# Tencent/PocketFlow

Hardware: AMD Instinct MI355X
Metric: images/sec ResNet-50 INT8 quant-aware fine-tune (whole job; per GPU = value / n_gpus) (higher is better)
Workload: dtype bf16

## Files before the change

### include/pocketflow_hip.h

```cpp
#ifndef POCKETFLOW_HIP_H_
#define POCKETFLOW_HIP_H_

#include <stdint.h>

#ifdef __cplusplus
extern "C" {
#endif

enum { PF_F32 = 0, PF_BF16 = 1 };
enum { PF_ACT_NONE = 0, PF_ACT_RELU = 1, PF_ACT_RELU6 = 2 };
enum { PF_BUCKET_TENSOR = 0, PF_BUCKET_CHANNEL = 1, PF_BUCKET_SPLIT = 2 };

typedef struct PfSeg {
  int64_t offset;
  int64_t len;
  int32_t RS;
  int32_t layout;
  int32_t I, O;
  int32_t mode;
  int32_t bits;
  int32_t bucket_size;
  int32_t n_bucket;
  int64_t slot_offset;
  int64_t cb_offset;
} PfSeg;

typedef struct PfBlock { int32_t seg; int32_t chunk; int32_t row0; int32_t nrows; } PfBlock;

#define PF_CHUNK 4096

const char* pf_error_string(int err);
int pf_version(void);
int pf_tuning_reload(void);

int pf_minmax_slots_init(uint32_t* slots, int64_t n_pairs, void* stream);
int pf_minmax_tensor(const void* x, int64_t n, int dtype, int act, uint32_t* slot, void* stream);
int pf_minmax_decode(const uint32_t* slots, int64_t n_pairs, float* alpha_beta, void* stream);

int pf_uq_apply(const void* x, void* y, int64_t n, int in_dtype, int out_dtype, int act,
                const uint32_t* slot, int bits, void* stream);
int pf_act_grad(const void* g, const void* u, void* dx, int64_t n, int dtype, int act,
                void* stream);

int pf_seg_minmax(const float* w_flat, const PfSeg* segs, const PfBlock* blocks, int n_blocks,
                  uint32_t* slots, void* stream);
int pf_seg_uq_apply(const float* w_flat, void* qw_flat, int out_dtype, const PfSeg* segs,
                    const PfBlock* blocks, int n_blocks, const uint32_t* slots, void* stream);

int pf_seg_nuq_apply(const float* w_flat, void* qw_flat, int out_dtype, uint8_t* idx_flat,
                     const float* codebooks, const PfSeg* segs, const PfBlock* blocks,
                     int n_blocks, const uint32_t* slots, void* stream);
int pf_seg_nuq_codebook_grad(const void* g_flat, int g_dtype, const uint8_t* idx_flat,
                             float* dcodebooks, int64_t* acc_ws, int64_t n_codebook, const PfSeg* segs,
                             const PfBlock* blocks, int n_blocks, const uint32_t* slots, void* stream);
int pf_seg_normalize(const float* w_flat, float* xn_out, const PfSeg* segs, int seg_index,
                     const uint32_t* slots, void* stream);

int pf_ws_bkup_merge_abs(const float* var, float* bkup, const float* mask, float* abs_out,
                         int64_t n, void* stream);
int pf_kth_largest_nonneg(const float* a, int64_t n, int64_t k_desc_index, float* out,
                          uint32_t* workspace, void* stream);
int pf_ws_mask_apply(float* var, const float* bkup, float* mask, const float* thr, int64_t n,
                     void* stream);
int pf_count_nonzero(const float* x, int64_t n, unsigned long long* out, void* stream);

int pf_cp_build_mask(float* mask, const uint8_t* keep_in, const uint8_t* keep_out, int O, int RS,
                     int I, void* stream);
int pf_cp_mask_grad(float* g, const uint8_t* keep_in, const uint8_t* keep_out, int O, int RS,
                    int I, void* stream);

int pf_adam_flat(float* p, const void* g, int g_dtype, float* m, float* v, const float* mask,
                 int64_t n, int64_t n_decay, float wd, float g_scale, float lr, float beta1,
                 float beta2, float eps, float beta1_power, float beta2_power, void* stream);
int pf_momentum_flat(float* p, const void* g, int g_dtype, float* acc, const float* mask,
                     int64_t n, int64_t n_decay, float wd, float g_scale, float lr, float momentum,
                     void* stream);
int pf_adam_flat_dev(float* p, const void* g, int g_dtype, float* m, float* v, const float* mask,
                     int64_t n, int64_t n_decay, float wd, float g_scale, const float* hp, float beta1,
                     float beta2, float eps, void* stream);
int pf_momentum_flat_dev(float* p, const void* g, int g_dtype, float* acc, const float* mask,
                         int64_t n, int64_t n_decay, float wd, float g_scale, const float* hp,
                         float momentum, void* stream);
int pf_set_floats(float* dst, float a, float b, float c, float d, void* stream);

int pf_ce_distill_fwd_bwd(const void* z_s, int zs_dtype, const float* labels, const void* z_t,
                          int zt_dtype, int B, int C, float tempr, float loss_w, float* losses,
                          void* dz_s, int dz_dtype, float* row_ws, void* stream);

int pf_ce_distill_head(const void* z_s, int zs_dtype, const float* labels, const void* z_t,
                       int zt_dtype, int B, int C, float tempr, float loss_w, float* losses ,
                       void* dz_hard, void* dz_soft, int dz_dtype, float* row_ws, void* stream);
int pf_ce_combine(const void* dz_hard, const void* dz_soft, const float* g0, const float* g1, void* dz,
                  int dtype, int64_t n, void* stream);

int pf_bn_stats(const void* x, int dtype, int64_t rows, int C, float* partial ,
                int n_blocks, void* stream);
int pf_bn_finalize(const float* partial, int n_blocks, int64_t rows, int C, const void* x_row0,
                   int dtype, const float* gamma, const float* beta, float* moving_mean,
                   float* moving_var, float momentum, float eps, int training ,
                   int act, float* scale_shift , float* mean_invstd ,
                   uint32_t* slot , void* stream);
int pf_bn_act_quant_apply(const void* x, void* q, int dtype, int64_t rows, int C,
                          const float* scale_shift, int act, const uint32_t* slot, int bits,
                          int quantize, void* stream);
int pf_bn_act_quant_pool(const void* x, void* pooled, int dtype, int64_t rows, int C,
                         const float* scale_shift, int act, const uint32_t* slot, int bits,
                         int quantize, int HW, void* stream);
int pf_bn_bwd_stats_pooled(const void* g, const void* x, int dtype, int64_t rows, int C, int HW,
                           const float* scale_shift, const float* mean_invstd, int act,
                           float* partial , int n_blocks, void* stream);
int pf_bn_bwd_apply_pooled(const void* g, const void* x, void* dx, int dtype, int64_t rows, int C, int HW,
                           const float* scale_shift, const float* mean_invstd,
                           const float* dgamma, const float* dbeta, int act, void* stream);
int pf_bn_bwd_stats(const void* dq, const void* x, int dtype, int64_t rows, int C,
                    const float* scale_shift, const float* mean_invstd, int act,
                    float* partial , int n_blocks, void* stream);
int pf_bn_bwd_finalize(const float* partial, int n_blocks, int C, float* dgamma, float* dbeta,
                       void* stream);
int pf_bn_bwd_apply(const void* dq, const void* x, void* dx, int dtype, int64_t rows, int C,
                    const float* scale_shift, const float* mean_invstd,
                    const float* dgamma, const float* dbeta, int act, void* stream);
int pf_bn_bwd_apply_add(const void* dq, const void* x, const void* addend, void* dx, int dtype,
                        int64_t rows, int C, const float* scale_shift, const float* mean_invstd,
                        const float* dgamma, const float* dbeta, int act, void* stream);
int pf_bn_eval_scale_shift(const float* gamma, const float* beta, const float* moving_mean,
                           const float* moving_var, float eps, int C, float* scale_shift,
                           void* stream);

int pf_bn_add_act_groups(int64_t rows, int C);
int pf_bn_add_act_fwd(const void* x, const void* r, void* u, int dtype, int64_t rows, int C, const float* scale_shift, int act,
                      uint32_t* slot, void* stream);
int pf_bn_add_act_bwd_gate(const void* dq, const void* x, const void* r, void* g, int dtype, int64_t rows, int C,
                           const float* scale_shift, const float* mean_invstd, int act, float* partial, void* stream);
int pf_bn_add_act_bwd_gate_add(const void* dq, const void* addend, const void* x, const void* r, void* g, int dtype, int64_t rows,
                               int C, const float* scale_shift, const float* mean_invstd, int act, float* partial, void* stream);

int pf_conv1x1_stats_groups_k(int M, int N, int K, int prologue);
int pf_conv1x1_fwd(const void* X, const void* W, void* Y, const void* R, const float* scale_shift,
                   int act, const uint32_t* slot, int bits, float* partial, int M, int N, int K,
                   int Ho, int Wo, int H, int Wd, int stride, int ymap, void* stream);
int pf_conv1x1_fwd_affine(const void* X, const void* W, void* Y, const float* scale_shift, int act,
                          const float* out_scale_shift, int out_act, int M, int N, int K, int Ho, int Wo, int H, int Wd,
                          int stride, void* stream);
int pf_conv1x1_bwd_data_bnstats(const void* dY, const void* Wt, void* dQ, const void* bn_x,
                                const float* bn_scale_shift, const float* bn_mean_invstd, int bn_act,
                                float* partial, int M, int N, int K, void* stream);
int pf_conv1x1_join_plan(int M, int N, int K, int with_stats);
int pf_conv1x1_bwd_data_join(const void* dY, const void* Wt, void* dQ, const void* R, int r_Ho, int r_Wo, int r_H, int r_W,
                             int r_stride, const void* bn_x, const float* bn_scale_shift, const float* bn_mean_invstd,
                             int bn_act, float* partial, int M, int N, int K, void* stream);
int pf_conv1x1_wrw_splits(int M, int N, int K);
int pf_conv1x1_wrw(const void* dY, const void* X, void* dW, int dw_dtype, float* workspace,
                   const float* scale_shift, int act, const uint32_t* slot, int bits, int M, int N,
                   int K, int Ho, int Wo, int H, int Wd, int stride, void* stream);

int pf_conv2d_stats_groups_geom(int imgs, int H, int Wd, int C, int N, int th, int tw, int stride, int pad_h, int pad_w,
                                int Ho, int Wo);
int pf_conv2d_fwd(const void* X, const void* W, void* Y, const void* zero, const void* R, float* partial,
                  const void* bn_x, const float* bn_scale_shift, const float* bn_mean_invstd, int bn_act,
                  int imgs, int H, int Wd, int C, int N, int th, int tw, int stride, int pad_h, int pad_w,
                  int Ho, int Wo, void* stream);
int pf_conv2d_fwd_affine(const void* X, const void* W, void* Y, const void* zero, const float* out_scale_shift, int out_act,
                         int imgs, int H, int Wd, int C, int N, int th, int tw, int stride, int pad_h, int pad_w, int Ho, int Wo,
                         void* stream);

int pf_conv2d_wrw_splits(int M, int N, int C, int taps);
int pf_conv2d_wrw(const void* dY, const void* X, void* dW, int dw_dtype, float* workspace, int imgs, int H, int Wd, int C,
                  int N, int th, int tw, int stride, int pad_h, int pad_w, int Ho, int Wo, void* stream);

typedef struct PfTransposeTile {
  int64_t src_off, dst_off;
  int32_t O, I, src_ld, dst_ld;
  int32_t o0, i0;
  int32_t reserved0, reserved1;
} PfTransposeTile;
int pf_seg_transpose(const void* src_flat, void* dst_flat, int dtype, const void* tiles, int n_tiles, void* stream);

int pf_maxpool_fwd(const void* x, void* y, void* idx, int dtype, int B, int H, int W, int C, int k, int stride,
                   int pad_h, int pad_w, int Ho, int Wo, void* stream);
int pf_maxpool_bwd(const void* dy, const void* idx, void* dx, int dtype, int B, int H, int W, int C, int k, int stride,
                   int pad_h, int pad_w, int Ho, int Wo, void* stream);

int pf_conv_stem_supported(int H, int Wd, int C, int N, int k, int stride, int pad);
int pf_conv_stem_fwd(const void* X, const void* W, void* Y, int imgs, int H, int Wd, void* stream);
int pf_conv_stem_wrw_slabs(int imgs, int H, int Wd);
int pf_conv_stem_wrw(const void* dY, const void* X, void* dW, int dw_dtype, float* workspace, int imgs, int H, int Wd,
                     void* stream);

int pf_conv_stem3_supported(int H, int Wd, int C, int N, int k, int stride, int pad_h, int pad_w, int Ho, int Wo);
int pf_conv_stem3_fwd(const void* X, const void* W, void* Y, int imgs, int H, int Wd, int N, int pad_h, int pad_w, int Ho, int Wo,
                      void* stream);
int pf_conv_stem3_wrw_slabs(int imgs, int H, int Wd, int N, int pad_h, int pad_w, int Ho, int Wo);
int pf_conv_stem3_wrw(const void* dY, const void* X, void* dW, int dw_dtype, float* workspace, int imgs, int H, int Wd, int N,
                      int pad_h, int pad_w, int Ho, int Wo, void* stream);

int pf_depthwise_supported(int C, int k, int stride);
int pf_depthwise_groups(int B, int Ho, int Wo, int C);
int pf_depthwise_fwd(const void* X, const void* W, void* Y, int dtype, float* partial, int B, int H, int Wd, int C, int k,
                     int stride, int pad_h, int pad_w, int Ho, int Wo, void* stream);
int pf_depthwise_bwd_data(const void* dY, const void* W, void* dX, int dtype, int B, int H, int Wd, int C, int k,
                          int stride, int pad_h, int pad_w, int Ho, int Wo, void* stream);
int pf_depthwise_wrw(const void* dY, const void* X, void* dW, int dtype, int dw_dtype, float* slabs, int B, int H, int Wd,
                     int C, int k, int stride, int pad_h, int pad_w, int Ho, int Wo, void* stream);

typedef struct PfImageDesc {
  int64_t offset;
  int32_t h, w;
  float scale_y, scale_x;
  int32_t off_y, off_x;
  int32_t flip;
  int32_t reserved;
} PfImageDesc;
int pf_image_resize_bilinear(const void* src, const PfImageDesc* desc, void* out, int out_dtype, int B, int OH,
                             int OW, float mean_r, float mean_g, float mean_b, void* stream);

int pf_conv2d_bwd_data_strided(const void* dY, const void* Wt, void* dX, const void* zero, int imgs, int H, int Wd, int C, int N,
                               int R, int S, int stride, int pad_h, int pad_w, int Ho, int Wo, void* stream);
int pf_conv2d_bwd_data_strided_stats_groups(int imgs, int H, int Wd, int C, int stride);
int pf_conv2d_bwd_data_strided_bnstats(const void* dY, const void* Wt, void* dX, const void* zero, const void* bn_x,
                                       const float* bn_scale_shift, const float* bn_mean_invstd, int bn_act, float* partial,
                                       int imgs, int H, int Wd, int C, int N, int R, int S, int stride, int pad_h, int pad_w,
                                       int Ho, int Wo, void* stream);

int pf_convg_small_splits(int M, int Nc, int K);
int pf_convg_fwd(const void* x, const void* w, const float* bias, void* y, int dtype, int imgs, int H, int W, int C, int N, int R,
                 int S, int stride, int pad_h, int pad_w, int Ho, int Wo, float* slab, int64_t slab_elems, void* stream);
int pf_convg_bwd_data(const void* dy, const void* w, void* dx, int dtype, int imgs, int H, int W, int C, int N, int R, int S,
                      int stride, int pad_h, int pad_w, int Ho, int Wo, float* slab, int64_t slab_elems, void* stream);
int pf_convg_wrw_splits(int imgs, int C, int N, int R, int S, int Ho, int Wo);
int pf_convg_wrw(const void* dy, const void* x, void* dw, int dtype, int dw_dtype, float* slab, int imgs, int H, int W, int C, int N,
                 int R, int S, int stride, int pad_h, int pad_w, int Ho, int Wo, void* stream);

int pf_conv_gather_fwd(const void* x, const void* w, const int32_t* gather, const float* bias, const void* res,
                       const float* scale_shift, int act, void* y, int dtype, int imgs, int H, int W, int C, int Ck, int N, int R,
                       int S, int stride, int pad_h, int pad_w, int Ho, int Wo, void* stream);

int pf_bn_act_quant_codes(const void* x, uint8_t* codes, int dtype, int64_t rows, int C, const float* scale_shift, int act,
                          const uint32_t* slot, int bits, float* alpha_beta, void* stream);
int pf_conv_i8_supported(int C, int N, int R, int S, int stride);
int pf_conv_i8_fwd(const uint8_t* x, const int8_t* w, const float* act_alpha_beta, int act_bits, const float* w_scale_beta,
                   const int32_t* w_tsum, const int32_t* w_tapsum, const void* res, void* y, int out_dtype, int imgs, int H, int W,
                   int C, int N, int R, int S, int stride, int pad_h, int pad_w, int Ho, int Wo, void* stream);

int pf_dw_i8_supported(int C, int k, int stride);
int pf_dw_i8_fwd(const uint8_t* x, const uint32_t* w_cols, const float* w_scale_beta, const float* act_alpha_beta, int act_bits, void* y,
                 int dtype, int B, int H, int W, int C, int stride, int pad_h, int pad_w, int Ho, int Wo, void* stream);

int pf_bn_act_quant_static(const void* x, void* out, int dtype, int out_kind, int64_t rows, int C, const float* scale_shift, int act,
                           const float* out_alpha_beta, int bits, void* stream);
int pf_conv_i8_fwd_q(const uint8_t* x, const int8_t* w, const float* act_alpha_beta, int act_bits, const float* w_scale_beta,
                     const int32_t* w_tsum, const int32_t* w_tapsum, const void* res, const float* out_scale_shift, int out_act,
                     const float* out_alpha_beta, int out_bits, void* out, int out_kind, int imgs, int H, int W, int C, int N, int R,
                     int S, int stride, int pad_h, int pad_w, int Ho, int Wo, void* stream);
int pf_dw_i8_fwd_q(const uint8_t* x, const uint32_t* w_cols, const float* w_scale_beta, const float* act_alpha_beta, int act_bits,
                   const float* out_scale_shift, int out_act, const float* out_alpha_beta, int out_bits, void* out, int out_kind, int B,
                   int H, int W, int C, int stride, int pad_h, int pad_w, int Ho, int Wo, void* stream);

int pf_im2col(const void* x, void* xcol, int imgs, int H, int W, int C, int R, int S, int stride, int pad_h, int pad_w, int Ho, int Wo,
              void* stream);
int pf_col2im(const void* dxcol, void* dx, int imgs, int H, int W, int C, int R, int S, int stride, int pad_h, int pad_w, int Ho, int Wo,
              void* stream);

int pf_prox_groups(int64_t rows, int I);
int pf_prox_norms(const float* w, const void* g, int g_dtype, float lr, int64_t rows, int I, float* partial, float* norms, void* stream);
int pf_prox_apply(float* w, const void* g, int g_dtype, float lr, int64_t rows, int I, const float* norms, const float* thr, void* stream);

int pf_cpr_gather(const void* x, int x_dtype, const void* y, int y_dtype, const int* pos, int crops, int B, int H, int W, int C, int OH, int OW,
                  int Co, int kh, int kw, int stride, int pad_t, int pad_l, float* P, float* Y, int64_t row0, void* stream);
int64_t pf_cpr_gram_ws(int C);
int pf_cpr_gram(const float* P, const float* Y, const int* idx, int64_t n, int kk, int C, int Co, const float* w, double* ws, int64_t ws_elems,
                float* xtx, float* xty, void* stream);
int pf_cpr_ista(const float* A, const float* b, const float* m0, float* m_ws, float* mask, int C, float gamma, float lr, int iters, int* nnz,
                void* stream);
int pf_cpr_lstsq_splits(int64_t N, int Kp, int Co);
int pf_cpr_lstsq_step(const float* P, int K, const int* kidx, const int* pos, int Kp, const float* Y, float* R, int64_t N, int Co, float* W,
                      float* m, float* v, float* part, float wd, float lr_t, float beta1, float beta2, float c1, float c2, float eps,
                      void* stream);
int pf_cpr_lstsq_resid(const float* P, int K, const int* kidx, int Kp, const float* W, const float* Y, float* R, int64_t N, int Co,
                       void* stream);

#ifdef __cplusplus
}
#endif
#endif
```

### pocketflow_amd/csrc/pf_optim.hip

```cpp
#include "pf_common.h"

template <typename TG> __device__ __forceinline__ void load4g(const TG* p, float* g);
template <> __device__ __forceinline__ void load4g<float>(const float* p, float* g) {
  float4 v = *reinterpret_cast<const float4*>(p);
  g[0] = v.x; g[1] = v.y; g[2] = v.z; g[3] = v.w;
}
template <> __device__ __forceinline__ void load4g<bf16_t>(const bf16_t* p, float* g) {
  uint2 v = *reinterpret_cast<const uint2*>(p);
  g[0] = __uint_as_float(v.x << 16); g[1] = __uint_as_float(v.x & 0xFFFF0000u);
  g[2] = __uint_as_float(v.y << 16); g[3] = __uint_as_float(v.y & 0xFFFF0000u);
}

__device__ __forceinline__ float eff_grad(float g, float p, float mask, bool decay, float wd,
                                          float g_scale) {
  float ge = g * g_scale;
  if (decay) ge = ge + wd * p;
  return ge * mask;
}

template <typename TG, bool MASK>
__global__ __launch_bounds__(PF_THREADS) void k_adam_flat(float* __restrict__ p, const TG* __restrict__ g,
                                                          float* __restrict__ m, float* __restrict__ v,
                                                          const float* __restrict__ mask, int64_t n,
                                                          int64_t n_decay, float wd, float g_scale,
                                                          float alpha_t, float omb1, float omb2,
                                                          float eps, const float* __restrict__ hp) {
  if (hp != nullptr) alpha_t = hp[0];
  const int64_t nv = n >> 2;
  for (int64_t i = (int64_t)blockIdx.x * PF_THREADS + threadIdx.x; i < nv;
       i += (int64_t)gridDim.x * PF_THREADS) {
    const int64_t e = i << 2;
    float gg[4], mk[4] = {1.f, 1.f, 1.f, 1.f};
    load4g<TG>(g + e, gg);
    float4 pp = *reinterpret_cast<float4*>(p + e);
    float4 mm = *reinterpret_cast<float4*>(m + e);
    float4 vv = *reinterpret_cast<float4*>(v + e);
    if (MASK) { float4 t = *reinterpret_cast<const float4*>(mask + e); mk[0] = t.x; mk[1] = t.y; mk[2] = t.z; mk[3] = t.w; }
    float pa[4] = {pp.x, pp.y, pp.z, pp.w}, ma[4] = {mm.x, mm.y, mm.z, mm.w}, va[4] = {vv.x, vv.y, vv.z, vv.w};
#pragma unroll
    for (int j = 0; j < 4; ++j) {
      const float ge = eff_grad(gg[j], pa[j], mk[j], (e + j) < n_decay, wd, g_scale);
      ma[j] = ma[j] + (ge - ma[j]) * omb1;
      va[j] = va[j] + (ge * ge - va[j]) * omb2;
      pa[j] = pa[j] - (ma[j] * alpha_t) / (sqrtf(va[j]) + eps);
    }
    *reinterpret_cast<float4*>(p + e) = make_float4(pa[0], pa[1], pa[2], pa[3]);
    *reinterpret_cast<float4*>(m + e) = make_float4(ma[0], ma[1], ma[2], ma[3]);
    *reinterpret_cast<float4*>(v + e) = make_float4(va[0], va[1], va[2], va[3]);
  }
  if (blockIdx.x == 0) {
    for (int64_t e = (nv << 2) + threadIdx.x; e < n; e += PF_THREADS) {
      const float mk = MASK ? mask[e] : 1.0f;
      const float ge = eff_grad(load_one<TG>(g + e), p[e], mk, e < n_decay, wd, g_scale);
      const float mn = m[e] + (ge - m[e]) * omb1;
      const float vn = v[e] + (ge * ge - v[e]) * omb2;
      m[e] = mn; v[e] = vn;
      p[e] = p[e] - (mn * alpha_t) / (sqrtf(vn) + eps);
    }
  }
}

static int adam_launch(float* p, const void* g, int g_dtype, float* m, float* v,
                       const float* mask, int64_t n, int64_t n_decay, float wd, float g_scale,
                       float lr, float beta1, float beta2, float eps, float beta1_power,
                       float beta2_power, const float* hp, void* stream) {
  if (n <= 0) return 0;
  if (!pf_aligned16(p) || !pf_aligned16(g) || !pf_aligned16(m) || !pf_aligned16(v) ||
      (mask && !pf_aligned16(mask)))
    return (int)hipErrorInvalidValue;
  const float alpha_t = lr * sqrtf(1.0f - beta2_power) / (1.0f - beta1_power);
  const float omb1 = 1.0f - beta1, omb2 = 1.0f - beta2;
  hipStream_t st = (hipStream_t)stream;
  const int grid = pf_grid_for(n, PF_THREADS * 4);
#define PF_AD(TG, MK) k_adam_flat<TG, MK><<<grid, PF_THREADS, 0, st>>>(p, (const TG*)g, m, v, mask, n, n_decay, wd, g_scale, alpha_t, omb1, omb2, eps, hp)
  if (g_dtype == PF_F32) { if (mask) PF_AD(float, true); else PF_AD(float, false); }
  else if (g_dtype == PF_BF16) { if (mask) PF_AD(bf16_t, true); else PF_AD(bf16_t, false); }
  else return (int)hipErrorInvalidValue;
#undef PF_AD
  PF_LAUNCH_CHECK();
  return 0;
}

extern "C" int pf_adam_flat(float* p, const void* g, int g_dtype, float* m, float* v,
                            const float* mask, int64_t n, int64_t n_decay, float wd, float g_scale,
                            float lr, float beta1, float beta2, float eps, float beta1_power,
                            float beta2_power, void* stream) {
  return adam_launch(p, g, g_dtype, m, v, mask, n, n_decay, wd, g_scale, lr, beta1, beta2, eps, beta1_power, beta2_power, nullptr,
                     stream);
}

extern "C" int pf_adam_flat_dev(float* p, const void* g, int g_dtype, float* m, float* v,
                                const float* mask, int64_t n, int64_t n_decay, float wd, float g_scale,
                                const float* hp, float beta1, float beta2, float eps, void* stream) {
  if (hp == nullptr) return (int)hipErrorInvalidValue;
  return adam_launch(p, g, g_dtype, m, v, mask, n, n_decay, wd, g_scale, 0.f, beta1, beta2, eps, 0.5f, 0.5f, hp, stream);
}

template <typename TG, bool MASK>
__global__ __launch_bounds__(PF_THREADS) void k_momentum_flat(float* __restrict__ p, const TG* __restrict__ g,
                                                              float* __restrict__ acc,
                                                              const float* __restrict__ mask, int64_t n,
                                                              int64_t n_decay, float wd, float g_scale,
                                                              float lr, float mu, const float* __restrict__ hp) {
  if (hp != nullptr) lr = hp[1];
  const int64_t nv = n >> 2;
  for (int64_t i = (int64_t)blockIdx.x * PF_THREADS + threadIdx.x; i < nv;
       i += (int64_t)gridDim.x * PF_THREADS) {
    const int64_t e = i << 2;
    float gg[4], mk[4] = {1.f, 1.f, 1.f, 1.f};
    load4g<TG>(g + e, gg);
    float4 pp = *reinterpret_cast<float4*>(p + e);
    float4 aa = *reinterpret_cast<float4*>(acc + e);
    if (MASK) { float4 t = *reinterpret_cast<const float4*>(mask + e); mk[0] = t.x; mk[1] = t.y; mk[2] = t.z; mk[3] = t.w; }
    float pa[4] = {pp.x, pp.y, pp.z, pp.w}, ac[4] = {aa.x, aa.y, aa.z, aa.w};
#pragma unroll
    for (int j = 0; j < 4; ++j) {
      const float ge = eff_grad(gg[j], pa[j], mk[j], (e + j) < n_decay, wd, g_scale);
      ac[j] = mu * ac[j] + ge;
      pa[j] = pa[j] - lr * ac[j];
    }
    *reinterpret_cast<float4*>(p + e) = make_float4(pa[0], pa[1], pa[2], pa[3]);
    *reinterpret_cast<float4*>(acc + e) = make_float4(ac[0], ac[1], ac[2], ac[3]);
  }
  if (blockIdx.x == 0) {
    for (int64_t e = (nv << 2) + threadIdx.x; e < n; e += PF_THREADS) {
      const float mk = MASK ? mask[e] : 1.0f;
      const float ge = eff_grad(load_one<TG>(g + e), p[e], mk, e < n_decay, wd, g_scale);
      const float a = mu * acc[e] + ge;
      acc[e] = a;
      p[e] = p[e] - lr * a;
    }
  }
}

static int momentum_launch(float* p, const void* g, int g_dtype, float* acc, const float* mask,
                           int64_t n, int64_t n_decay, float wd, float g_scale, float lr,
                           float momentum, const float* hp, void* stream) {
  if (n <= 0) return 0;
  if (!pf_aligned16(p) || !pf_aligned16(g) || !pf_aligned16(acc) || (mask && !pf_aligned16(mask)))
    return (int)hipErrorInvalidValue;
  hipStream_t st = (hipStream_t)stream;
  const int grid = pf_grid_for(n, PF_THREADS * 4);
#define PF_MO(TG, MK) k_momentum_flat<TG, MK><<<grid, PF_THREADS, 0, st>>>(p, (const TG*)g, acc, mask, n, n_decay, wd, g_scale, lr, momentum, hp)
  if (g_dtype == PF_F32) { if (mask) PF_MO(float, true); else PF_MO(float, false); }
  else if (g_dtype == PF_BF16) { if (mask) PF_MO(bf16_t, true); else PF_MO(bf16_t, false); }
  else return (int)hipErrorInvalidValue;
#undef PF_MO
  PF_LAUNCH_CHECK();
  return 0;
}

extern "C" int pf_momentum_flat(float* p, const void* g, int g_dtype, float* acc, const float* mask,
                                int64_t n, int64_t n_decay, float wd, float g_scale, float lr,
                                float momentum, void* stream) {
  return momentum_launch(p, g, g_dtype, acc, mask, n, n_decay, wd, g_scale, lr, momentum, nullptr, stream);
}

extern "C" int pf_momentum_flat_dev(float* p, const void* g, int g_dtype, float* acc, const float* mask,
                                    int64_t n, int64_t n_decay, float wd, float g_scale, const float* hp,
                                    float momentum, void* stream) {
  if (hp == nullptr) return (int)hipErrorInvalidValue;
  return momentum_launch(p, g, g_dtype, acc, mask, n, n_decay, wd, g_scale, 0.f, momentum, hp, stream);
}

__global__ void k_set_floats(float* __restrict__ dst, float a, float b, float c, float d) {
  if (threadIdx.x == 0) { dst[0] = a; dst[1] = b; dst[2] = c; dst[3] = d; }
}

extern "C" int pf_set_floats(float* dst, float a, float b, float c, float d, void* stream) {
  if (dst == nullptr) return (int)hipErrorInvalidValue;
  k_set_floats<<<1, 64, 0, (hipStream_t)stream>>>(dst, a, b, c, d);
  PF_LAUNCH_CHECK();
  return 0;
}
```

### pocketflow_amd/csrc/pf_pool.hip

```cpp
#include "pf_common.h"
#include <stdlib.h>

template <typename T>
__global__ __launch_bounds__(PF_THREADS) void k_maxpool_fwd(const T* __restrict__ x, T* __restrict__ y,
                                                            uint8_t* __restrict__ idx, int B, int H, int W, int C,
                                                            int k, int stride, int pad_h, int pad_w, int Ho, int Wo) {
  const int CV = C >> 3;
  const int64_t total = (int64_t)B * Ho * Wo * CV;
  for (int64_t e = (int64_t)blockIdx.x * PF_THREADS + threadIdx.x; e < total; e += (int64_t)gridDim.x * PF_THREADS) {
    const int cv = (int)(e % CV);
    int64_t p = e / CV;
    const int wo = (int)(p % Wo); p /= Wo;
    const int ho = (int)(p % Ho);
    const int b = (int)(p / Ho);
    float best[8];
    int arg[8];
#pragma unroll
    for (int j = 0; j < 8; ++j) { best[j] = -INFINITY; arg[j] = 0; }
    for (int r = 0; r < k; ++r) {
      const int hi = ho * stride + r - pad_h;
      if ((unsigned)hi >= (unsigned)H) continue;
      for (int s = 0; s < k; ++s) {
        const int wi = wo * stride + s - pad_w;
        if ((unsigned)wi >= (unsigned)W) continue;
        float v[8];
        load8<T>(x + (((int64_t)b * H + hi) * W + wi) * C + (cv << 3), v);
#pragma unroll
        for (int j = 0; j < 8; ++j)
          if (v[j] > best[j] || v[j] != v[j]) { best[j] = v[j]; arg[j] = r * k + s; }
      }
    }
    const int64_t o = (((int64_t)b * Ho + ho) * Wo + wo) * C + (cv << 3);
    store8<T>(y + o, best);
    if (idx != nullptr) {
      uint2 pk;
      pk.x = (uint32_t)arg[0] | ((uint32_t)arg[1] << 8) | ((uint32_t)arg[2] << 16) | ((uint32_t)arg[3] << 24);
      pk.y = (uint32_t)arg[4] | ((uint32_t)arg[5] << 8) | ((uint32_t)arg[6] << 16) | ((uint32_t)arg[7] << 24);
      *reinterpret_cast<uint2*>(idx + o) = pk;
    }
  }
}

template <typename T>
__global__ __launch_bounds__(PF_THREADS) void k_maxpool_bwd(const T* __restrict__ dy, const uint8_t* __restrict__ idx,
                                                            T* __restrict__ dx, int B, int H, int W, int C, int k,
                                                            int stride, int pad_h, int pad_w, int Ho, int Wo) {
  const int CV = C >> 3;
  const int64_t total = (int64_t)B * H * W * CV;
  for (int64_t e = (int64_t)blockIdx.x * PF_THREADS + threadIdx.x; e < total; e += (int64_t)gridDim.x * PF_THREADS) {
    const int cv = (int)(e % CV);
    int64_t p = e / CV;
    const int wi = (int)(p % W); p /= W;
    const int hi = (int)(p % H);
    const int b = (int)(p / H);
    float g[8];
#pragma unroll
    for (int j = 0; j < 8; ++j) g[j] = 0.f;
    const int ho_hi = (hi + pad_h) / stride;
    const int wo_hi = (wi + pad_w) / stride;
    for (int ho = ho_hi; ho >= 0 && ho * stride - pad_h + k - 1 >= hi; --ho) {
      if (ho >= Ho) continue;
      const int r = hi - (ho * stride - pad_h);
      for (int wo = wo_hi; wo >= 0 && wo * stride - pad_w + k - 1 >= wi; --wo) {
        if (wo >= Wo) continue;
        const int s = wi - (wo * stride - pad_w);
        const int64_t o = (((int64_t)b * Ho + ho) * Wo + wo) * C + (cv << 3);
        const uint2 pk = *reinterpret_cast<const uint2*>(idx + o);
        float d[8];
        load8<T>(dy + o, d);
        const uint32_t want = (uint32_t)(r * k + s);
#pragma unroll
        for (int j = 0; j < 8; ++j) {
          const uint32_t a = ((j < 4 ? pk.x : pk.y) >> ((j & 3) * 8)) & 0xFFu;
          if (a == want) g[j] += d[j];
        }
      }
    }
    store8<T>(dx + (((int64_t)b * H + hi) * W + wi) * C + (cv << 3), g);
  }
}

template <typename T>
__global__ __launch_bounds__(PF_THREADS) void k_maxpool3s2_fwd(const T* __restrict__ x, T* __restrict__ y,
                                                               uint8_t* __restrict__ idx, int B, int H, int W, int C,
                                                               int pad_h, int pad_w, int Ho, int Wo) {
  const int CV = C >> 3;
  const int total = B * Ho * Wo * CV;
  for (int64_t e64 = (int64_t)blockIdx.x * PF_THREADS + threadIdx.x; e64 < total; e64 += (int64_t)gridDim.x * PF_THREADS) {
    const int e = (int)e64;
    const int cv = e % CV;
    int p = e / CV;
    const int wo = p % Wo; p /= Wo;
    const int ho = p % Ho;
    const int b = p / Ho;
    const int h0 = ho * 2 - pad_h, w0 = wo * 2 - pad_w;
    float v[9][8];
#pragma unroll
    for (int r = 0; r < 3; ++r)
#pragma unroll
      for (int s = 0; s < 3; ++s) {
        const int hi = h0 + r, wi = w0 + s;
        const int hc = hi < 0 ? 0 : (hi >= H ? H - 1 : hi), wc = wi < 0 ? 0 : (wi >= W ? W - 1 : wi);
        load8<T>(x + (((int64_t)b * H + hc) * W + wc) * C + (cv << 3), v[r * 3 + s]);
      }
#pragma unroll
    for (int r = 0; r < 3; ++r)
#pragma unroll
      for (int s = 0; s < 3; ++s) {
        const bool ok = (unsigned)(h0 + r) < (unsigned)H && (unsigned)(w0 + s) < (unsigned)W;
#pragma unroll
        for (int j = 0; j < 8; ++j) v[r * 3 + s][j] = ok ? v[r * 3 + s][j] : -INFINITY;
      }
    float best[8];
    int arg[8];
#pragma unroll
    for (int j = 0; j < 8; ++j) { best[j] = -INFINITY; arg[j] = 0; }
#pragma unroll
    for (int t = 0; t < 9; ++t)
#pragma unroll
      for (int j = 0; j < 8; ++j)
        if (v[t][j] > best[j] || v[t][j] != v[t][j]) { best[j] = v[t][j]; arg[j] = t; }
    const int64_t o = (((int64_t)b * Ho + ho) * Wo + wo) * C + (cv << 3);
    store8<T>(y + o, best);
    if (idx != nullptr) {
      uint2 pk;
      pk.x = (uint32_t)arg[0] | ((uint32_t)arg[1] << 8) | ((uint32_t)arg[2] << 16) | ((uint32_t)arg[3] << 24);
      pk.y = (uint32_t)arg[4] | ((uint32_t)arg[5] << 8) | ((uint32_t)arg[6] << 16) | ((uint32_t)arg[7] << 24);
      *reinterpret_cast<uint2*>(idx + o) = pk;
    }
  }
}

template <typename T>
__global__ __launch_bounds__(PF_THREADS) void k_maxpool3s2_bwd(const T* __restrict__ dy, const uint8_t* __restrict__ idx,
                                                               T* __restrict__ dx, int B, int H, int W, int C, int pad_h,
                                                               int pad_w, int Ho, int Wo, int Ha, int Wb) {
  const int CV = C >> 3;
  const int total = B * Ha * Wb * CV;
  for (int64_t e64 = (int64_t)blockIdx.x * PF_THREADS + threadIdx.x; e64 < total; e64 += (int64_t)gridDim.x * PF_THREADS) {
    const int e = (int)e64;
    const int cv = e % CV;
    int p = e / CV;
    const int bb = p % Wb; p /= Wb;
    const int a = p % Ha;
    const int b = p / Ha;
    float d[2][2][8];
    uint2 pk[2][2];
#pragma unroll
    for (int i = 0; i < 2; ++i)
#pragma unroll
      for (int k = 0; k < 2; ++k) {
        const int ho = a - i, wo = bb - k;
        const bool ok = (unsigned)ho < (unsigned)Ho && (unsigned)wo < (unsigned)Wo;
        const int hoc = ho < 0 ? 0 : (ho >= Ho ? Ho - 1 : ho), woc = wo < 0 ? 0 : (wo >= Wo ? Wo - 1 : wo);
        const int64_t o = (((int64_t)b * Ho + hoc) * Wo + woc) * C + (cv << 3);
        const uint2 pki = *reinterpret_cast<const uint2*>(idx + o);
        load8<T>(dy + o, d[i][k]);
        pk[i][k] = ok ? pki : make_uint2(0xFFFFFFFFu, 0xFFFFFFFFu);
      }
#pragma unroll
    for (int du = 0; du < 2; ++du) {
      const int hi = 2 * a + du - pad_h;
      if ((unsigned)hi >= (unsigned)H) continue;
#pragma unroll
      for (int dv = 0; dv < 2; ++dv) {
        const int wi = 2 * bb + dv - pad_w;
        if ((unsigned)wi >= (unsigned)W) continue;
        float g[8];
#pragma unroll
        for (int j = 0; j < 8; ++j) g[j] = 0.f;
#pragma unroll
        for (int i = 0; i < 2; ++i) {
          const int r = du + 2 * i;
          if (r > 2) continue;
#pragma unroll
          for (int k = 0; k < 2; ++k) {
            const int s = dv + 2 * k;
            if (s > 2) continue;
            const uint32_t want = (uint32_t)(r * 3 + s);
#pragma unroll
            for (int j = 0; j < 8; ++j) {
              const uint32_t t = ((j < 4 ? pk[i][k].x : pk[i][k].y) >> ((j & 3) * 8)) & 0xFFu;
              if (t == want) g[j] += d[i][k][j];
            }
          }
        }
        store8<T>(dx + (((int64_t)b * H + hi) * W + wi) * C + (cv << 3), g);
      }
    }
  }
}

static bool pool3s2_ok(int B, int H, int W, int C, int k, int stride, int pad_h, int pad_w, int Ho, int Wo) {
  if (pf_tuning().pool3s2 == 0) return false;
  return k == 3 && stride == 2 && pad_h >= 0 && pad_h <= 1 && pad_w >= 0 && pad_w <= 1 &&
         (int64_t)B * H * W * (C / 8) < (1ll << 31);
}

extern "C" int pf_maxpool_fwd(const void* x, void* y, void* idx, int dtype, int B, int H, int W, int C, int k, int stride,
                              int pad_h, int pad_w, int Ho, int Wo, void* stream) {
  if (B <= 0 || H <= 0 || W <= 0 || C <= 0 || (C % 8) || k < 1 || k > 15 || stride < 1 || Ho <= 0 || Wo <= 0)
    return (int)hipErrorInvalidValue;
  if (!pf_aligned16(x) || !pf_aligned16(y) || (idx && (((uintptr_t)idx) & 7))) return (int)hipErrorInvalidValue;
  const int64_t total = (int64_t)B * Ho * Wo * (C / 8);
  const int grid = pf_grid_for(total, PF_THREADS);
  hipStream_t st = (hipStream_t)stream;
  if (pool3s2_ok(B, H, W, C, k, stride, pad_h, pad_w, Ho, Wo) && (dtype == PF_F32 || dtype == PF_BF16)) {
    if (dtype == PF_F32)
      k_maxpool3s2_fwd<float><<<grid, PF_THREADS, 0, st>>>((const float*)x, (float*)y, (uint8_t*)idx, B, H, W, C, pad_h, pad_w, Ho, Wo);
    else
      k_maxpool3s2_fwd<bf16_t><<<grid, PF_THREADS, 0, st>>>((const bf16_t*)x, (bf16_t*)y, (uint8_t*)idx, B, H, W, C, pad_h, pad_w, Ho, Wo);
    PF_LAUNCH_CHECK();
    return 0;
  }
  if (dtype == PF_F32)
    k_maxpool_fwd<float><<<grid, PF_THREADS, 0, st>>>((const float*)x, (float*)y, (uint8_t*)idx, B, H, W, C, k, stride,
                                                       pad_h, pad_w, Ho, Wo);
  else if (dtype == PF_BF16)
    k_maxpool_fwd<bf16_t><<<grid, PF_THREADS, 0, st>>>((const bf16_t*)x, (bf16_t*)y, (uint8_t*)idx, B, H, W, C, k, stride,
                                                        pad_h, pad_w, Ho, Wo);
  else
    return (int)hipErrorInvalidValue;
  PF_LAUNCH_CHECK();
  return 0;
}

extern "C" int pf_maxpool_bwd(const void* dy, const void* idx, void* dx, int dtype, int B, int H, int W, int C, int k,
                              int stride, int pad_h, int pad_w, int Ho, int Wo, void* stream) {
  if (B <= 0 || H <= 0 || W <= 0 || C <= 0 || (C % 8) || k < 1 || k > 15 || stride < 1 || Ho <= 0 || Wo <= 0 || idx == nullptr)
    return (int)hipErrorInvalidValue;
  if (!pf_aligned16(dy) || !pf_aligned16(dx) || (((uintptr_t)idx) & 7)) return (int)hipErrorInvalidValue;
  const int64_t total = (int64_t)B * H * W * (C / 8);
  hipStream_t st = (hipStream_t)stream;
  if (pool3s2_ok(B, H, W, C, k, stride, pad_h, pad_w, Ho, Wo) && (dtype == PF_F32 || dtype == PF_BF16)) {
    const int Ha = (H + pad_h + 1) / 2, Wb = (W + pad_w + 1) / 2;
    const int g2 = pf_grid_for((int64_t)B * Ha * Wb * (C / 8), PF_THREADS);
    if (dtype == PF_F32)
      k_maxpool3s2_bwd<float><<<g2, PF_THREADS, 0, st>>>((const float*)dy, (const uint8_t*)idx, (float*)dx, B, H, W, C, pad_h, pad_w, Ho, Wo, Ha, Wb);
    else
      k_maxpool3s2_bwd<bf16_t><<<g2, PF_THREADS, 0, st>>>((const bf16_t*)dy, (const uint8_t*)idx, (bf16_t*)dx, B, H, W, C, pad_h, pad_w, Ho, Wo, Ha, Wb);
    PF_LAUNCH_CHECK();
    return 0;
  }
  const int grid = pf_grid_for(total, PF_THREADS);
  if (dtype == PF_F32)
    k_maxpool_bwd<float><<<grid, PF_THREADS, 0, st>>>((const float*)dy, (const uint8_t*)idx, (float*)dx, B, H, W, C, k,
                                                       stride, pad_h, pad_w, Ho, Wo);
  else if (dtype == PF_BF16)
    k_maxpool_bwd<bf16_t><<<grid, PF_THREADS, 0, st>>>((const bf16_t*)dy, (const uint8_t*)idx, (bf16_t*)dx, B, H, W, C, k,
                                                        stride, pad_h, pad_w, Ho, Wo);
  else
    return (int)hipErrorInvalidValue;
  PF_LAUNCH_CHECK();
  return 0;
}
```

### pocketflow_amd/csrc/pf_quant.hip

```cpp
#include "pf_common.h"

template <typename T, int ACT, bool VEC>
__global__ __launch_bounds__(PF_THREADS) void k_minmax_tensor(const T* __restrict__ x, int64_t n,
                                                              uint32_t* __restrict__ slot) {
  __shared__ float lds[8];
  float mn = INFINITY, mx = -INFINITY;
  const int64_t tid = (int64_t)blockIdx.x * PF_THREADS + threadIdx.x;
  const int64_t stride = (int64_t)gridDim.x * PF_THREADS;
  int64_t done = 0;
  if (VEC) {
    const int64_t nv = n >> 3;
#pragma unroll 2
    for (int64_t i = tid; i < nv; i += stride) {
      float v[8];
      load8<T>(x + (i << 3), v);
#pragma unroll
      for (int j = 0; j < 8; ++j) {
        float t = apply_act<ACT>(v[j]);
        mn = fminf(mn, t);
        mx = fmaxf(mx, t);
      }
    }
    done = nv << 3;
  }
  for (int64_t i = done + tid; i < n; i += stride) {
    float t = apply_act<ACT>(load_one<T>(x + i));
    mn = fminf(mn, t);
    mx = fmaxf(mx, t);
  }
  block_minmax(mn, mx, lds);
  if (threadIdx.x == 0 && mn <= mx) {
    atomicMin(&slot[0], enc_f32(mn));
    atomicMin(&slot[1], ~enc_f32(mx));
  }
}

template <typename T, bool VEC>
static void launch_minmax_tensor(const T* x, int64_t n, int act, uint32_t* slot, hipStream_t st) {
  const int grid = pf_grid_for(n, PF_THREADS * 16);
  switch (act) {
    case PF_ACT_RELU: k_minmax_tensor<T, PF_ACT_RELU, VEC><<<grid, PF_THREADS, 0, st>>>(x, n, slot); break;
    case PF_ACT_RELU6: k_minmax_tensor<T, PF_ACT_RELU6, VEC><<<grid, PF_THREADS, 0, st>>>(x, n, slot); break;
    default: k_minmax_tensor<T, PF_ACT_NONE, VEC><<<grid, PF_THREADS, 0, st>>>(x, n, slot); break;
  }
}

extern "C" int pf_minmax_slots_init(uint32_t* slots, int64_t n_pairs, void* stream) {
  if (n_pairs <= 0) return 0;
  return (int)hipMemsetAsync(slots, 0xFF, (size_t)n_pairs * 2 * sizeof(uint32_t), (hipStream_t)stream);
}

extern "C" int pf_minmax_tensor(const void* x, int64_t n, int dtype, int act, uint32_t* slot,
                                void* stream) {
  if (n <= 0) return 0;
  if (dtype != PF_F32 && dtype != PF_BF16) return (int)hipErrorInvalidValue;
  hipStream_t st = (hipStream_t)stream;
  const bool vec = pf_aligned16(x);
  if (dtype == PF_F32) {
    if (vec) launch_minmax_tensor<float, true>((const float*)x, n, act, slot, st);
    else launch_minmax_tensor<float, false>((const float*)x, n, act, slot, st);
  } else {
    if (vec) launch_minmax_tensor<bf16_t, true>((const bf16_t*)x, n, act, slot, st);
    else launch_minmax_tensor<bf16_t, false>((const bf16_t*)x, n, act, slot, st);
  }
  PF_LAUNCH_CHECK();
  return 0;
}

__global__ void k_minmax_decode(const uint32_t* __restrict__ slots, int64_t n_pairs,
                                float* __restrict__ ab) {
  const int64_t i = (int64_t)blockIdx.x * blockDim.x + threadIdx.x;
  if (i < n_pairs) {
    float a, b;
    slot_alpha_beta(slots + 2 * i, a, b);
    ab[2 * i] = a;
    ab[2 * i + 1] = b;
  }
}
extern "C" int pf_minmax_decode(const uint32_t* slots, int64_t n_pairs, float* alpha_beta,
                                void* stream) {
  if (n_pairs <= 0) return 0;
  k_minmax_decode<<<(int)((n_pairs + 255) / 256), 256, 0, (hipStream_t)stream>>>(slots, n_pairs, alpha_beta);
  PF_LAUNCH_CHECK();
  return 0;
}

template <typename TI, typename TO, int ACT, bool VEC>
__global__ __launch_bounds__(PF_THREADS) void k_uq_apply(const TI* __restrict__ x, TO* __restrict__ y,
                                                         int64_t n, const uint32_t* __restrict__ slot,
                                                         float k) {
  float alpha, beta;
  slot_alpha_beta(slot, alpha, beta);
  const int64_t tid = (int64_t)blockIdx.x * PF_THREADS + threadIdx.x;
  const int64_t stride = (int64_t)gridDim.x * PF_THREADS;
  int64_t done = 0;
  if (VEC) {
    const int64_t nv = n >> 3;
#pragma unroll 2
    for (int64_t i = tid; i < nv; i += stride) {
      float v[8];
      load8<TI>(x + (i << 3), v);
#pragma unroll
      for (int j = 0; j < 8; ++j) v[j] = uq_point(apply_act<ACT>(v[j]), alpha, beta, k);
      store8<TO>(y + (i << 3), v);
    }
    done = nv << 3;
  }
  for (int64_t i = done + tid; i < n; i += stride)
    store_one<TO>(y + i, uq_point(apply_act<ACT>(load_one<TI>(x + i)), alpha, beta, k));
}

template <typename TI, typename TO, bool VEC>
static void launch_uq_apply(const TI* x, TO* y, int64_t n, int act, const uint32_t* slot, float k,
                            hipStream_t st) {
  const int grid = pf_grid_for(n, PF_THREADS * 16);
  switch (act) {
    case PF_ACT_RELU: k_uq_apply<TI, TO, PF_ACT_RELU, VEC><<<grid, PF_THREADS, 0, st>>>(x, y, n, slot, k); break;
    case PF_ACT_RELU6: k_uq_apply<TI, TO, PF_ACT_RELU6, VEC><<<grid, PF_THREADS, 0, st>>>(x, y, n, slot, k); break;
    default: k_uq_apply<TI, TO, PF_ACT_NONE, VEC><<<grid, PF_THREADS, 0, st>>>(x, y, n, slot, k); break;
  }
}

extern "C" int pf_uq_apply(const void* x, void* y, int64_t n, int in_dtype, int out_dtype, int act,
                           const uint32_t* slot, int bits, void* stream) {
  if (n <= 0) return 0;
  if (bits < 1 || bits > 32) return (int)hipErrorInvalidValue;
  hipStream_t st = (hipStream_t)stream;
  const float k = uq_k_of_bits(bits);
  const bool vec = pf_aligned16(x) && pf_aligned16(y);
#define PF_DISPATCH(TI, TO)                                                     \
  do {                                                                          \
    if (vec) launch_uq_apply<TI, TO, true>((const TI*)x, (TO*)y, n, act, slot, k, st);  \
    else launch_uq_apply<TI, TO, false>((const TI*)x, (TO*)y, n, act, slot, k, st);     \
  } while (0)
  if (in_dtype == PF_F32 && out_dtype == PF_F32) PF_DISPATCH(float, float);
  else if (in_dtype == PF_F32 && out_dtype == PF_BF16) PF_DISPATCH(float, bf16_t);
  else if (in_dtype == PF_BF16 && out_dtype == PF_BF16) PF_DISPATCH(bf16_t, bf16_t);
  else if (in_dtype == PF_BF16 && out_dtype == PF_F32) PF_DISPATCH(bf16_t, float);
  else return (int)hipErrorInvalidValue;
#undef PF_DISPATCH
  PF_LAUNCH_CHECK();
  return 0;
}

template <typename T, int ACT, bool VEC>
__global__ __launch_bounds__(PF_THREADS) void k_act_grad(const T* __restrict__ g, const T* __restrict__ u,
                                                         T* __restrict__ dx, int64_t n) {
  const int64_t tid = (int64_t)blockIdx.x * PF_THREADS + threadIdx.x;
  const int64_t stride = (int64_t)gridDim.x * PF_THREADS;
  int64_t done = 0;
  if (VEC) {
    const int64_t nv = n >> 3;
#pragma unroll 2
    for (int64_t i = tid; i < nv; i += stride) {
      float a[8], b[8];
      load8<T>(g + (i << 3), a);
      load8<T>(u + (i << 3), b);
#pragma unroll
      for (int j = 0; j < 8; ++j) a[j] = a[j] * act_mask<ACT>(b[j]);
      store8<T>(dx + (i << 3), a);
    }
    done = nv << 3;
  }
  for (int64_t i = done + tid; i < n; i += stride)
    store_one<T>(dx + i, load_one<T>(g + i) * act_mask<ACT>(load_one<T>(u + i)));
}

template <typename T>
static int launch_act_grad(const T* g, const T* u, T* dx, int64_t n, int act, hipStream_t st) {
  const int grid = pf_grid_for(n, PF_THREADS * 16);
  const bool vec = pf_aligned16(g) && pf_aligned16(u) && pf_aligned16(dx);
  pf_with_act(act, [&](auto A) {
    pf_with_bool(vec, [&](auto V) {
      k_act_grad<T, decltype(A)::value, decltype(V)::value><<<grid, PF_THREADS, 0, st>>>(g, u, dx, n);
    });
  });
  PF_LAUNCH_CHECK();
  return 0;
}

extern "C" int pf_act_grad(const void* g, const void* u, void* dx, int64_t n, int dtype, int act,
                           void* stream) {
  if (n <= 0) return 0;
  if (dtype == PF_F32) return launch_act_grad<float>((const float*)g, (const float*)u, (float*)dx, n, act, (hipStream_t)stream);
  if (dtype == PF_BF16) return launch_act_grad<bf16_t>((const bf16_t*)g, (const bf16_t*)u, (bf16_t*)dx, n, act, (hipStream_t)stream);
  return (int)hipErrorInvalidValue;
}


__device__ __forceinline__ uint32_t hwio_flat_index(const PfSeg& sg, uint32_t e) {
  if (sg.layout == 0) {
    const uint32_t L = (uint32_t)sg.RS * (uint32_t)sg.I;
    const uint32_t o = e / L;
    const uint32_t rem = e - o * L;
    return rem * (uint32_t)sg.O + o;
  }
  const uint32_t i = e / (uint32_t)sg.RS;
  const uint32_t rs = e - i * (uint32_t)sg.RS;
  return rs * (uint32_t)sg.I + i;
}

__global__ __launch_bounds__(PF_THREADS) void k_seg_minmax(const float* __restrict__ w,
                                                           const PfSeg* __restrict__ segs,
                                                           const PfBlock* __restrict__ blocks,
                                                           uint32_t* __restrict__ slots) {
  __shared__ float lds[8];
  const PfBlock b = blocks[blockIdx.x];
  const PfSeg sg = segs[b.seg];
  const float* __restrict__ base = w + sg.offset;
  uint32_t* __restrict__ sl = slots + 2 * sg.slot_offset;

  if (sg.mode == PF_BUCKET_CHANNEL) {
    const int wave = threadIdx.x >> 6, lane = threadIdx.x & 63;
    const int row = b.chunk * 4 + wave;
    if (row >= sg.O) return;
    const int64_t L = (int64_t)sg.RS * sg.I;
    const float* __restrict__ r = base + (int64_t)row * L;
    float mn = INFINITY, mx = -INFINITY;
    if ((L & 3) == 0) {
      for (int64_t i = lane * 4; i < L; i += 256) {
        float4 v = *reinterpret_cast<const float4*>(r + i);
        mn = fminf(fminf(mn, v.x), fminf(v.y, fminf(v.z, v.w)));
        mx = fmaxf(fmaxf(mx, v.x), fmaxf(v.y, fmaxf(v.z, v.w)));
      }
    } else {
      for (int64_t i = lane; i < L; i += 64) { float v = r[i]; mn = fminf(mn, v); mx = fmaxf(mx, v); }
    }
    mn = wave_min(mn);
    mx = wave_max(mx);
    if (lane == 0) { sl[2 * row] = enc_f32(mn); sl[2 * row + 1] = ~enc_f32(mx); }
    return;
  }

  const int64_t e0 = (int64_t)b.chunk * PF_CHUNK;
  if (sg.mode == PF_BUCKET_SPLIT) {
    const uint32_t m = (uint32_t)sg.n_bucket;
    __shared__ uint32_t bins[2 * 1024];
    const bool use_bins = m <= 1024u;
    if (use_bins) {
      for (uint32_t j = threadIdx.x; j < 2 * m; j += PF_THREADS) bins[j] = 0xFFFFFFFFu;
      __syncthreads();
    }
    for (int t = threadIdx.x; t < PF_CHUNK; t += PF_THREADS) {
      const int64_t e = e0 + t;
      if (e < sg.len) {
        const float v = base[e];
        const uint32_t j = hwio_flat_index(sg, (uint32_t)e) % m;
        if (use_bins) {
          atomicMin(&bins[2 * j], enc_f32(v));
          atomicMin(&bins[2 * j + 1], ~enc_f32(v));
        } else {
          atomicMin(&sl[2 * j], enc_f32(v));
          atomicMin(&sl[2 * j + 1], ~enc_f32(v));
        }
      }
    }
    if (use_bins) {
      __syncthreads();
      for (uint32_t j = threadIdx.x; j < 2 * m; j += PF_THREADS)
        if (bins[j] != 0xFFFFFFFFu) atomicMin(&sl[j], bins[j]);
    }
    if (b.chunk == 0) {
      const float last = base[sg.len - 1];
      const uint32_t total = m * (uint32_t)sg.bucket_size;
      for (uint32_t f = (uint32_t)sg.len + threadIdx.x; f < total; f += PF_THREADS) {
        const uint32_t j = f % m;
        atomicMin(&sl[2 * j], enc_f32(last));
        atomicMin(&sl[2 * j + 1], ~enc_f32(last));
      }
    }
    return;
  }

  float mn = INFINITY, mx = -INFINITY;
#pragma unroll
  for (int it = 0; it < 4; ++it) {
    const int64_t e = e0 + it * 1024 + threadIdx.x * 4;
    if (e + 3 < sg.len) {
      float4 v = *reinterpret_cast<const float4*>(base + e);
      mn = fminf(fminf(mn, v.x), fminf(v.y, fminf(v.z, v.w)));
      mx = fmaxf(fmaxf(mx, v.x), fmaxf(v.y, fmaxf(v.z, v.w)));
    } else {
      for (int j = 0; j < 4; ++j)
        if (e + j < sg.len) { float v = base[e + j]; mn = fminf(mn, v); mx = fmaxf(mx, v); }
    }
  }
  block_minmax(mn, mx, lds);
  if (threadIdx.x == 0 && mn <= mx) {
    atomicMin(&sl[0], enc_f32(mn));
    atomicMin(&sl[1], ~enc_f32(mx));
  }
}

extern "C" int pf_seg_minmax(const float* w_flat, const PfSeg* segs, const PfBlock* blocks,
                             int n_blocks, uint32_t* slots, void* stream) {
  if (n_blocks <= 0) return 0;
  k_seg_minmax<<<n_blocks, PF_THREADS, 0, (hipStream_t)stream>>>(w_flat, segs, blocks, slots);
  PF_LAUNCH_CHECK();
  return 0;
}

#define PF_LDS_ROWS 1024

template <typename TO> __device__ __forceinline__ void store4(TO* p, const float* v);
template <> __device__ __forceinline__ void store4<float>(float* p, const float* v) {
  *reinterpret_cast<float4*>(p) = make_float4(v[0], v[1], v[2], v[3]);
}
template <> __device__ __forceinline__ void store4<bf16_t>(bf16_t* p, const float* v) {
  uint2 o;
  o.x = (uint32_t)f32_to_bf16(v[0]) | ((uint32_t)f32_to_bf16(v[1]) << 16);
  o.y = (uint32_t)f32_to_bf16(v[2]) | ((uint32_t)f32_to_bf16(v[3]) << 16);
  *reinterpret_cast<uint2*>(p) = o;
}

__device__ __forceinline__ int nuq_argmin(float xn, const float* __restrict__ c, int k, int cs) {
  int best = 0;
  float bd = fabsf(xn - c[0]);
  for (int j = 1; j < k; ++j) {
    const float d = fabsf(xn - c[(int64_t)j * cs]);
    if (d < bd) { bd = d; best = j; }
  }
  return best;
}

template <typename TO, bool NUQ>
__global__ __launch_bounds__(PF_THREADS) void k_seg_apply(const float* __restrict__ w, TO* __restrict__ qw,
                                                          uint8_t* __restrict__ idx_out,
                                                          const float* __restrict__ codebooks,
                                                          const PfSeg* __restrict__ segs,
                                                          const PfBlock* __restrict__ blocks,
                                                          const uint32_t* __restrict__ slots) {
  __shared__ float s_alpha[PF_LDS_ROWS];
  __shared__ float s_beta[PF_LDS_ROWS];
  __shared__ float s_cb[NUQ ? 4096 : 1];
  const PfBlock b = blocks[blockIdx.x];
  const PfSeg sg = segs[b.seg];
  const float* __restrict__ base = w + sg.offset;
  TO* __restrict__ out = qw + sg.offset;
  const uint32_t* __restrict__ sl = slots + 2 * sg.slot_offset;
  const uint32_t e0 = (uint32_t)b.chunk * PF_CHUNK;
  const uint32_t L = (uint32_t)sg.RS * (uint32_t)sg.I;
  const uint32_t len = (uint32_t)sg.len;
  const float kf = uq_k_of_bits(sg.bits);
  const int kc = NUQ ? (1 << sg.bits) : 0;
  const float* __restrict__ cb = NUQ ? (codebooks + sg.cb_offset) : nullptr;

  int row0 = 0, nrows = 1;
  bool in_lds = true;
  if (sg.mode == PF_BUCKET_CHANNEL) {
    row0 = b.row0;
    nrows = b.nrows;
    in_lds = nrows <= PF_LDS_ROWS;
  } else if (sg.mode == PF_BUCKET_SPLIT) {
    in_lds = false;
  }
  if (in_lds) {
#pragma unroll
    for (int q = 0; q < PF_LDS_ROWS / PF_THREADS; ++q) {
      const int r = threadIdx.x + q * PF_THREADS;
      if (r < nrows) {
        float a, bt;
        slot_alpha_beta(sl + 2 * (row0 + r), a, bt);
        s_alpha[r] = a;
        s_beta[r] = bt;
      }
    }
  }
  bool cb_lds = false;
  if (NUQ) {
    if (sg.mode == PF_BUCKET_TENSOR) {
      cb_lds = true;
      for (int j = threadIdx.x; j < kc; j += PF_THREADS) s_cb[j] = cb[j];
    } else if (sg.mode == PF_BUCKET_CHANNEL && in_lds && nrows * kc <= 4096) {
      cb_lds = true;
      for (int t = threadIdx.x; t < nrows * kc; t += PF_THREADS) {
        const int r = t / kc, j = t - r * kc;
        s_cb[t] = cb[(int64_t)j * sg.n_bucket + row0 + r];
      }
    }
  }
  __syncthreads();

#pragma unroll
  for (int it = 0; it < 4; ++it) {
    const uint32_t e = e0 + it * 1024 + threadIdx.x * 4;
    if (e >= len) continue;
    float v[4];
    const bool full = (e + 3 < len);
    if (full) {
      float4 t = *reinterpret_cast<const float4*>(base + e);
      v[0] = t.x; v[1] = t.y; v[2] = t.z; v[3] = t.w;
    } else {
      for (int j = 0; j < 4; ++j) v[j] = (e + j < len) ? base[e + j] : 0.0f;
    }
    uint32_t packed_idx = 0;
#pragma unroll
    for (int j = 0; j < 4; ++j) {
      const uint32_t ej = e + j;
      float alpha, beta;
      uint32_t bucket = 0;
      if (sg.mode == PF_BUCKET_TENSOR) {
        alpha = s_alpha[0]; beta = s_beta[0];
      } else if (sg.mode == PF_BUCKET_CHANNEL) {
        bucket = ej / L;
        if (bucket > (uint32_t)sg.O - 1) bucket = (uint32_t)sg.O - 1;
        if (in_lds) { alpha = s_alpha[bucket - row0]; beta = s_beta[bucket - row0]; }
        else slot_alpha_beta(sl + 2 * bucket, alpha, beta);
      } else {
        bucket = (ej < len ? hwio_flat_index(sg, ej) : 0u) % (uint32_t)sg.n_bucket;
        slot_alpha_beta(sl + 2 * bucket, alpha, beta);
      }
      if (sg.bits <= 0) {
      } else if (!NUQ) {
        v[j] = uq_point(v[j], alpha, beta, kf);
      } else {
        const float xn = (v[j] - beta) / alpha;
        int best;
        float cval;
        if (cb_lds) {
          const float* c = (sg.mode == PF_BUCKET_TENSOR) ? s_cb : (s_cb + (bucket - row0) * kc);
          best = nuq_argmin(xn, c, kc, 1);
          cval = c[best];
        } else {
          const float* c = cb + bucket;
          best = nuq_argmin(xn, c, kc, sg.n_bucket);
          cval = c[(int64_t)best * sg.n_bucket];
        }
        const float s = xn + 1e-6f;
        const float sgn = (s > 0.0f) ? 1.0f : ((s < 0.0f) ? -1.0f : 0.0f);
        const float q = cval * sgn;
        v[j] = alpha * q + beta;
        packed_idx |= ((uint32_t)best) << (8 * j);
      }
    }
    if (full) {
      store4<TO>(out + e, v);
      if (NUQ) *reinterpret_cast<uint32_t*>(idx_out + sg.offset + e) = packed_idx;
    } else {
      for (int j = 0; j < 4; ++j)
        if (e + j < len) {
          store_one<TO>(out + e + j, v[j]);
          if (NUQ) idx_out[sg.offset + e + j] = (uint8_t)((packed_idx >> (8 * j)) & 0xFF);
        }
    }
  }
}

extern "C" int pf_seg_uq_apply(const float* w_flat, void* qw_flat, int out_dtype, const PfSeg* segs,
                               const PfBlock* blocks, int n_blocks, const uint32_t* slots,
                               void* stream) {
  if (n_blocks <= 0) return 0;
  hipStream_t st = (hipStream_t)stream;
  if (out_dtype == PF_F32)
    k_seg_apply<float, false><<<n_blocks, PF_THREADS, 0, st>>>(w_flat, (float*)qw_flat, nullptr, nullptr, segs, blocks, slots);
  else if (out_dtype == PF_BF16)
    k_seg_apply<bf16_t, false><<<n_blocks, PF_THREADS, 0, st>>>(w_flat, (bf16_t*)qw_flat, nullptr, nullptr, segs, blocks, slots);
  else return (int)hipErrorInvalidValue;
  PF_LAUNCH_CHECK();
  return 0;
}

extern "C" int pf_seg_nuq_apply(const float* w_flat, void* qw_flat, int out_dtype, uint8_t* idx_flat,
                                const float* codebooks, const PfSeg* segs, const PfBlock* blocks,
                                int n_blocks, const uint32_t* slots, void* stream) {
  if (n_blocks <= 0) return 0;
  hipStream_t st = (hipStream_t)stream;
  if (out_dtype == PF_F32)
    k_seg_apply<float, true><<<n_blocks, PF_THREADS, 0, st>>>(w_flat, (float*)qw_flat, idx_flat, codebooks, segs, blocks, slots);
  else if (out_dtype == PF_BF16)
    k_seg_apply<bf16_t, true><<<n_blocks, PF_THREADS, 0, st>>>(w_flat, (bf16_t*)qw_flat, idx_flat, codebooks, segs, blocks, slots);
  else return (int)hipErrorInvalidValue;
  PF_LAUNCH_CHECK();
  return 0;
}

#define PF_CB_FX_SCALE 68719476736.0
__device__ __forceinline__ long long cb_to_fx(float v) { return __double2ll_rn((double)v * PF_CB_FX_SCALE); }

template <typename TG>
__global__ __launch_bounds__(PF_THREADS) void k_seg_nuq_cbgrad(const TG* __restrict__ g,
                                                               const uint8_t* __restrict__ idx,
                                                               unsigned long long* __restrict__ acc,
                                                               const PfSeg* __restrict__ segs,
                                                               const PfBlock* __restrict__ blocks,
                                                               const uint32_t* __restrict__ slots) {
  __shared__ unsigned long long bins[256];
  const PfBlock b = blocks[blockIdx.x];
  const PfSeg sg = segs[b.seg];
  if (sg.bits <= 0) return;
  const TG* __restrict__ gb = g + sg.offset;
  const uint8_t* __restrict__ ib = idx + sg.offset;
  const uint32_t* __restrict__ sl = slots + 2 * sg.slot_offset;
  unsigned long long* __restrict__ dc = acc + sg.cb_offset;
  const int kc = 1 << sg.bits;
  const uint32_t e0 = (uint32_t)b.chunk * PF_CHUNK;
  const uint32_t L = (uint32_t)sg.RS * (uint32_t)sg.I;
  const bool tensor_mode = (sg.mode == PF_BUCKET_TENSOR);
  if (tensor_mode) {
    for (int j = threadIdx.x; j < kc; j += PF_THREADS) bins[j] = 0ull;
    __syncthreads();
  }
  float alpha0 = 0.f, beta0 = 0.f;
  if (tensor_mode) slot_alpha_beta(sl, alpha0, beta0);
  for (int t = threadIdx.x; t < PF_CHUNK; t += PF_THREADS) {
    const uint32_t e = e0 + t;
    if (e >= (uint32_t)sg.len) break;
    const float gv = load_one<TG>(gb + e);
    const int j = ib[e];
    if (tensor_mode) {
      atomicAdd(&bins[j], (unsigned long long)cb_to_fx(alpha0 * gv));
    } else {
      uint32_t bucket;
      if (sg.mode == PF_BUCKET_CHANNEL) bucket = e / L;
      else bucket = hwio_flat_index(sg, e) % (uint32_t)sg.n_bucket;
      float a, bt;
      slot_alpha_beta(sl + 2 * bucket, a, bt);
      atomicAdd(&dc[(int64_t)j * sg.n_bucket + bucket], (unsigned long long)cb_to_fx(a * gv));
    }
  }
  if (tensor_mode) {
    __syncthreads();
    for (int j = threadIdx.x; j < kc; j += PF_THREADS)
      if (bins[j] != 0ull) atomicAdd(&dc[j], bins[j]);
  }
}

__global__ __launch_bounds__(PF_THREADS) void k_cb_fx_to_float(const long long* __restrict__ acc, float* __restrict__ dcb,
                                                               int64_t n) {
  for (int64_t i = (int64_t)blockIdx.x * PF_THREADS + threadIdx.x; i < n; i += (int64_t)gridDim.x * PF_THREADS)
    dcb[i] += (float)((double)acc[i] * (1.0 / PF_CB_FX_SCALE));
}

extern "C" int pf_seg_nuq_codebook_grad(const void* g_flat, int g_dtype, const uint8_t* idx_flat,
                                        float* dcodebooks, int64_t* acc_ws, int64_t n_codebook, const PfSeg* segs,
                                        const PfBlock* blocks, int n_blocks, const uint32_t* slots, void* stream) {
  if (n_blocks <= 0) return 0;
  if (acc_ws == nullptr || n_codebook <= 0) return (int)hipErrorInvalidValue;
  hipStream_t st = (hipStream_t)stream;
  hipError_t me = hipMemsetAsync(acc_ws, 0, (size_t)n_codebook * sizeof(int64_t), st);
  if (me != hipSuccess) return (int)me;
  unsigned long long* acc = reinterpret_cast<unsigned long long*>(acc_ws);
  if (g_dtype == PF_F32)
    k_seg_nuq_cbgrad<float><<<n_blocks, PF_THREADS, 0, st>>>((const float*)g_flat, idx_flat, acc, segs, blocks, slots);
  else if (g_dtype == PF_BF16)
    k_seg_nuq_cbgrad<bf16_t><<<n_blocks, PF_THREADS, 0, st>>>((const bf16_t*)g_flat, idx_flat, acc, segs, blocks, slots);
  else return (int)hipErrorInvalidValue;
  PF_LAUNCH_CHECK();
  k_cb_fx_to_float<<<pf_grid_for(n_codebook, PF_THREADS), PF_THREADS, 0, st>>>((const long long*)acc_ws, dcodebooks, n_codebook);
  PF_LAUNCH_CHECK();
  return 0;
}
```

### pocketflow_amd/csrc/pf_transpose.hip

```cpp
#include "pf_common.h"

struct PfTile {
  int64_t src_off;
  int64_t dst_off;
  int32_t O, I;
  int32_t src_ld, dst_ld;
  int32_t o0, i0;
  int32_t pad0, pad1;
};

template <typename T>
__global__ __launch_bounds__(PF_THREADS) void k_seg_transpose(const T* __restrict__ src, T* __restrict__ dst,
                                                              const PfTile* __restrict__ tiles) {
  __shared__ T tile[64][65];
  const PfTile t = tiles[blockIdx.x];
  const int tx = threadIdx.x & 63, ty = threadIdx.x >> 6;
#pragma unroll 4
  for (int r = ty; r < 64; r += 4) {
    const int o = t.o0 + r, i = t.i0 + tx;
    if (o < t.O && i < t.I) tile[r][tx] = src[t.src_off + (int64_t)o * t.src_ld + i];
  }
  __syncthreads();
#pragma unroll 4
  for (int r = ty; r < 64; r += 4) {
    const int i = t.i0 + r, o = t.o0 + tx;
    if (o < t.O && i < t.I) dst[t.dst_off + (int64_t)i * t.dst_ld + o] = tile[tx][r];
  }
}

extern "C" int pf_seg_transpose(const void* src_flat, void* dst_flat, int dtype, const void* tiles, int n_tiles,
                                void* stream) {
  if (n_tiles <= 0) return 0;
  hipStream_t st = (hipStream_t)stream;
  if (dtype == PF_F32)
    k_seg_transpose<float><<<n_tiles, PF_THREADS, 0, st>>>((const float*)src_flat, (float*)dst_flat, (const PfTile*)tiles);
  else if (dtype == PF_BF16)
    k_seg_transpose<bf16_t><<<n_tiles, PF_THREADS, 0, st>>>((const bf16_t*)src_flat, (bf16_t*)dst_flat, (const PfTile*)tiles);
  else
    return (int)hipErrorInvalidValue;
  PF_LAUNCH_CHECK();
  return 0;
}
```

### pocketflow_amd/graph.py

```python
from __future__ import annotations

import contextlib
import math
import os
import threading
from dataclasses import dataclass, field
from typing import Callable, Dict, List, Optional, Sequence, Tuple

import numpy as np
import torch
import torch.nn.functional as F

from pocketflow_amd import hip
from pocketflow_amd.hip import check_gather
from pocketflow_amd.plan import WeightDesc
from pocketflow_amd.profiling import region

ALIGN = 64
FUSE_BN_BWD_STATS = os.environ.get('PF_FUSE_BN_BWD_STATS', '1') != '0'
HEAD_FUSE = os.environ.get('PF_HEAD_FUSE', '1') != '0'
HEAD_FUSE_ANY_DEVICE = False
BN_JOIN_ANY_DEVICE = False
BN_TRAIN, BN_EVAL_GRAD, BN_EVAL = 0, 1, 2


def _align(n: int) -> int:
  return (n + ALIGN - 1) // ALIGN * ALIGN



@dataclass
class Variable:
  name: str
  ref_shape: Tuple[int, ...]
  kind: str
  trainable: bool = True
  l2: bool = True
  init: Optional[Callable[[np.random.RandomState], np.ndarray]] = field(default=None, repr=False)
  group: str = ''
  offset: int = 0
  numel: int = 0
  tensor: Optional[torch.Tensor] = field(default=None, repr=False)
  store: Optional[object] = field(default=None, repr=False)
  master: Optional[torch.Tensor] = field(default=None, repr=False)
  cin_full: int = 0
  gather_host: Optional[np.ndarray] = field(default=None, repr=False)
  gather: Optional[torch.Tensor] = field(default=None, repr=False)

  @property
  def storage_shape(self) -> Tuple[int, ...]:
    s = self.ref_shape
    if self.kind == 'conv':
      return (s[3], s[0], s[1], s[2])
    if self.kind == 'dense':
      return (s[1], s[0])
    if self.kind == 'depthwise':
      return (s[2], s[0], s[1])
    return tuple(s)

  def to_storage(self, ref: np.ndarray) -> np.ndarray:
    ref = np.asarray(ref, dtype=np.float32).reshape(self.ref_shape)
    if self.kind == 'conv':
      return np.ascontiguousarray(ref.transpose(3, 0, 1, 2))
    if self.kind == 'dense':
      return np.ascontiguousarray(ref.T)
    if self.kind == 'depthwise':
      return np.ascontiguousarray(ref[:, :, :, 0].transpose(2, 0, 1))
    return ref

  def to_ref(self, st: np.ndarray) -> np.ndarray:
    st = np.asarray(st, dtype=np.float32).reshape(self.storage_shape)
    if self.kind == 'conv':
      return np.ascontiguousarray(st.transpose(1, 2, 3, 0))
    if self.kind == 'dense':
      return np.ascontiguousarray(st.T)
    if self.kind == 'depthwise':
      return np.ascontiguousarray(st.transpose(1, 2, 0)[:, :, :, None])
    return st

  def weight_desc(self) -> WeightDesc:
    s = self.ref_shape
    if self.kind == 'conv':
      return WeightDesc(self.name, self.offset, s[0] * s[1], s[2], s[3], 0)
    if self.kind == 'dense':
      return WeightDesc(self.name, self.offset, 1, s[0], s[1], 0)
    if self.kind == 'depthwise':
      return WeightDesc(self.name, self.offset, s[0] * s[1], s[2], 1, 1)
    raise ValueError('not a matmul kernel: %s' % self.name)


class VarStore:

  def __init__(self, scope: str):
    self.scope = scope
    self.vars: List[Variable] = []
    self.by_name: Dict[str, Variable] = {}
    self.finalized = False
    self.device = None
    self.compute_dtype = torch.float32
    self.weight_decay = 0.0
    self.grad_hook = None

  def add(self, name: str, ref_shape, kind: str, trainable: bool = True, l2: bool = True,
          init=None) -> Variable:
    full = self.scope + '/' + name if self.scope else name
    if full in self.by_name:
      return self.by_name[full]
    if self.finalized:
      raise RuntimeError('variable %s created after the store was finalized' % full)
    v = Variable(full, tuple(int(d) for d in ref_shape), kind, trainable, l2 and trainable, init)
    v.numel = int(np.prod(v.ref_shape))
    v.group = 'W' if kind in ('conv', 'dense', 'depthwise') else ('O' if trainable else 'S')
    v.store = self
    self.vars.append(v)
    self.by_name[full] = v
    return v

  @property
  def trainable_vars(self) -> List[Variable]:
    return [v for v in self.vars if v.trainable]

  @property
  def matmul_vars(self) -> List[Variable]:
    return [v for v in self.vars if v.group == 'W']

  def notify_grad(self, var: 'Variable') -> None:
    if self.grad_hook is not None:
      self.grad_hook(var)

  def finalize(self, device, compute_dtype=torch.float32, separate_compute: bool = False,
               seed: int = 42, requires_grad: bool = True) -> None:
    if self.finalized:
      return
    self.device = torch.device(device)
    self.compute_dtype = compute_dtype
    separate_compute = separate_compute or compute_dtype != torch.float32
    self.separate_compute = separate_compute
    off = 0
    for flag in (True, False):
      for v in self.vars:
        if v.group == 'W' and v.l2 == flag:
          v.offset = off
          off += _align(v.numel)
      if flag:
        self.w_decay = off
    self.w_size = off
    off = 0
    for flag in (True, False):
      for v in self.vars:
        if v.group == 'O' and v.l2 == flag:
          v.offset = off
          off += _align(v.numel)
      if flag:
        self.o_decay = off
    self.o_size = off
    off = 0
    for v in self.vars:
      if v.group == 'S':
        v.offset = off
        off += _align(v.numel)
    self.s_size = off
    dev = self.device
    self.w_master = torch.zeros(max(self.w_size, ALIGN), dtype=torch.float32, device=dev)
    self.w_compute = (torch.zeros(max(self.w_size, ALIGN), dtype=compute_dtype, device=dev)
                      if separate_compute else self.w_master)
    self.o_master = torch.zeros(max(self.o_size, ALIGN), dtype=torch.float32, device=dev)
    self.state = torch.zeros(max(self.s_size, ALIGN), dtype=torch.float32, device=dev)
    self.w_grad = torch.zeros_like(self.w_compute) if requires_grad else None
    self.w_t = None
    self.w_t_fresh = False
    self._t_tiles, self._n_t_tiles = None, 0
    self.o_grad = torch.zeros_like(self.o_master) if requires_grad else None
    for v in self.vars:
      n = v.numel
      if v.group == 'W':
        v.master = self.w_master[v.offset:v.offset + n].view(v.storage_shape)
        t = self.w_compute[v.offset:v.offset + n].view(v.storage_shape)
        if v.kind == 'conv':
          t = t.permute(0, 3, 1, 2)
        elif v.kind == 'depthwise':
          t = t.unsqueeze(1)
        if requires_grad and v.trainable:
          t = t.detach().requires_grad_(True)
          g = self.w_grad[v.offset:v.offset + n].view(v.storage_shape)
          if v.kind == 'conv':
            g = g.permute(0, 3, 1, 2)
          elif v.kind == 'depthwise':
            g = g.unsqueeze(1)
          t.grad = g
          t.register_post_accumulate_grad_hook(lambda _t, _v=v: self.notify_grad(_v))
        v.tensor = t
      elif v.group == 'O':
        v.master = self.o_master[v.offset:v.offset + n].view(v.storage_shape)
        t = v.master
        if requires_grad:
          t = t.detach().requires_grad_(True)
          t.grad = self.o_grad[v.offset:v.offset + n].view(v.storage_shape)
        v.tensor = t
      else:
        v.master = self.state[v.offset:v.offset + n].view(v.storage_shape)
        v.tensor = v.master
    self.finalized = True
    self.initialize(seed)

  def initialize(self, seed: int = 42) -> None:
    rng = np.random.RandomState(seed)
    vals = {}
    for v in self.vars:
      if v.init is not None:
        vals[v.name] = v.init(rng)
    self.load_numpy(vals, strict=False)

  def load_numpy(self, values: Dict[str, np.ndarray], strict: bool = True, rename_scope: str = None) -> None:
    for v in self.vars:
      key = v.name
      if rename_scope is not None:
        key = rename_scope + '/' + '/'.join(v.name.split('/')[1:])
      if key not in values:
        if strict:
          raise KeyError('variable %s missing from checkpoint' % key)
        continue
      st = torch.from_numpy(v.to_storage(values[key])).to(self.device)
      v.master.copy_(st)
    self.sync_compute()

  def export_numpy(self) -> Dict[str, np.ndarray]:
    out = {}
    for v in self.vars:
      out[v.name] = v.to_ref(v.master.detach().float().cpu().numpy())
    return out

  def sync_compute(self) -> None:
    if self.separate_compute:
      self.w_compute.copy_(self.w_master)
    self.w_t_fresh = False

  def _build_transpose_tiles(self) -> None:
    rows = []
    for v in self.vars:
      if v.group != 'W' or v.kind != 'conv':
        continue
      kh, kw, cin, cout = v.ref_shape
      RS = kh * kw
      for rs in range(RS):
        for o0 in range(0, cout, 64):
          for i0 in range(0, cin, 64):
            rows.append((v.offset + rs * cin, v.offset + (RS - 1 - rs) * cout, cout, cin, RS * cin, RS * cout, o0, i0, 0, 0))
    from pocketflow_amd.hip import TILE_DTYPE
    tiles = np.array(rows, dtype=TILE_DTYPE) if rows else np.zeros(0, dtype=TILE_DTYPE)
    self._n_t_tiles = len(rows)
    self._t_tiles = torch.from_numpy(tiles.view(np.uint8).copy()).to(self.device) if rows else None
    self.w_t = torch.zeros_like(self.w_compute)

  def transposed(self, v: 'Variable') -> torch.Tensor:
    if self.w_t is None:
      self._build_transpose_tiles()
    if not self.w_t_fresh:
      if self._n_t_tiles:
        hip.seg_transpose(self.w_compute, self.w_t, self._t_tiles, self._n_t_tiles)
      self.w_t_fresh = True
    kh, kw, cin, cout = v.ref_shape
    return self.w_t[v.offset:v.offset + v.numel].view(cin, kh, kw, cout)

  def zero_grad(self) -> None:
    if self.w_grad is not None:
      self.w_grad.zero_()
      self.o_grad.zero_()

  def weight_descs(self, variables: Sequence[Variable]) -> List[WeightDesc]:
    return [v.weight_desc() for v in variables]

  def l2_loss_sum(self) -> torch.Tensor:
    tot = torch.zeros((), dtype=torch.float32, device=self.device)
    for v in self.vars:
      if v.trainable and v.l2:
        tot = tot + 0.5 * (v.master.float() ** 2).sum()
    return tot



@dataclass
class MatmulOp:
  type: str
  name: str
  var: Variable
  flops_per_out: int = 0


@dataclass
class ActivationOp:
  type: str
  name: str
  index: int = 0
  bits: Optional[int] = None


_tls = threading.local()


def get_default_graph() -> 'Graph':
  g = getattr(_tls, 'graph', None)
  if g is None:
    raise RuntimeError('no default Graph: call forward functions inside `with graph.as_default():`')
  return g


class Graph:

  def __init__(self, scope: str = 'model', device='cuda', compute_dtype=torch.float32):
    self.scope = scope
    self.device = torch.device(device)
    self.compute_dtype = compute_dtype
    self.store = VarStore(scope)
    self.matmul_ops: List[MatmulOp] = []
    self.activation_ops: List[ActivationOp] = []
    self.nets: Dict[str, object] = {}
    self.capturing = False
    self.step_feeders: List = []
    self.training = True
    self.frozen = False
    self.act_slots: Optional[torch.Tensor] = None
    self._scratch: Optional[torch.Tensor] = None
    self._zero_row: Optional[torch.Tensor] = None
    self.fuse_conv1x1 = True
    self.taps: Optional[Dict[object, tuple]] = None
    self.tap_dense = False
    self.tap_stop = None
    self._names: Dict[str, int] = {}
    self.reinflated: List[str] = []
    self.kernel_params = self.kernel_params_kept = self.nb_gathered = 0
    self.int8 = False
    self.nb_int8 = 0
    self.int8_ran: set = set()
    self.act_static: Optional[torch.Tensor] = None
    self.requant_ran: set = set()
    self._identity_ss: Dict[int, torch.Tensor] = {}
    self.conv_layers: List = []
    self.depthwise_layers: List = []
    self.join_layers: List = []

  def unique_name(self, base: str) -> str:
    k = self._names.get(base, 0)
    self._names[base] = k + 1
    return base if k == 0 else '%s_%d' % (base, k)

  def as_default(self):
    graph = self

    class _Ctx:
      def __enter__(self_inner):
        self_inner.prev = getattr(_tls, 'graph', None)
        _tls.graph = graph
        return graph

      def __exit__(self_inner, *exc):
        _tls.graph = self_inner.prev
        return False
    return _Ctx()

  def add_matmul_op(self, op_type: str, name: str, var: Variable) -> MatmulOp:
    op = MatmulOp(op_type, self.scope + '/' + name, var)
    self.matmul_ops.append(op)
    return op

  def add_activation_op(self, op_type: str, name: str) -> ActivationOp:
    op = ActivationOp(op_type, self.scope + '/' + name, len(self.activation_ops))
    self.activation_ops.append(op)
    return op

  def apply_gathers(self, gathers: Dict[str, np.ndarray], values: Optional[Dict[str, np.ndarray]] = None) -> None:
    if self.store.finalized:
      raise RuntimeError('apply_gathers: the graph is already finalised')
    for name, vec in gathers.items():
      var = self.store.by_name.get(name)
      if var is None:
        raise ValueError('%s: gather for a variable this graph does not have' % name)
      if var.kind != 'conv':
        raise ValueError('%s: a gather applies to Conv2D kernels only, this is a %s variable' % (name, var.kind))
      if var.gather_host is not None:
        raise ValueError('%s: the kernel already has a gather' % name)
      kh, kw, cin, cout = var.ref_shape
      g = check_gather(vec, cin, int(np.asarray(vec).size), what=name)
      if cin > GATHER_MAX_CIN:
        raise ValueError('%s: %d input channels, the gather kernel takes at most %d' % (name, cin, GATHER_MAX_CIN))
      shape = (kh, kw, int(g.size), cout)
      if values is not None and name in values and tuple(np.shape(values[name])) != shape:
        raise ValueError('%s: kernel of shape %s does not match its gather of %d kept channels (expected %s)'
                         % (name, tuple(np.shape(values[name])), g.size, shape))
      full_init = var.init
      var.cin_full, var.gather_host, var.ref_shape, var.numel = cin, g, shape, int(np.prod(shape))
      if full_init is not None:
        var.init = lambda rng, _f=full_init, _g=g: np.ascontiguousarray(_f(rng)[:, :, _g, :])

  def finalize(self, separate_compute: bool = False, seed: int = 42, requires_grad: bool = True) -> None:
    self.store.finalize(self.device, self.compute_dtype, separate_compute, seed, requires_grad)
    for v in self.store.vars:
      if v.gather_host is not None and v.gather is None:
        v.gather = torch.from_numpy(v.gather_host).to(self.device)
    n_act = max(len(self.activation_ops), 1)
    self.act_slots = torch.empty((n_act, 2), dtype=torch.int32, device=self.device)

  def begin_step(self) -> None:
    hip.minmax_slots_init(self.act_slots)
    self.store.w_t_fresh = False

  def scratch(self, n_floats: int) -> torch.Tensor:
    if self._scratch is None or self._scratch.numel() < n_floats:
      self._scratch = torch.empty(max(n_floats, 1 << 20), dtype=torch.float32, device=self.device)
    return self._scratch

  def act_alpha_beta(self) -> torch.Tensor:
    return hip.minmax_decode(self.act_slots)

  def identity_scale_shift(self, C: int) -> torch.Tensor:
    ss = self._identity_ss.get(C)
    if ss is None:
      ss = self._identity_ss[C] = torch.cat([torch.ones(C, dtype=torch.float32), torch.zeros(C, dtype=torch.float32)]).view(2, C).to(self.device)
    return ss

  def zero_row(self, C: int) -> torch.Tensor:
    if self._zero_row is None or self._zero_row.numel() < C:
      self._zero_row = torch.zeros(max(C, 4096), dtype=torch.float32, device=self.device)
    return self._zero_row



WRW_SIDE = os.environ.get('PF_WRW_SIDE', '1') != '0'


class WrwSide(object):

  def __init__(self, device):
    self.device = device
    self.stream = torch.cuda.Stream(device=device)
    self.keep: List = []
    self._scratch: Optional[torch.Tensor] = None
    self.armed = False
    self.forks = 0

  def scratch(self, n_floats: int) -> torch.Tensor:
    if self._scratch is None or self._scratch.numel() < n_floats:
      with torch.cuda.stream(self.stream):
        self._scratch = torch.empty(max(n_floats, 1 << 20), dtype=torch.float32, device=self.device)
    return self._scratch

  def join(self) -> None:
    if self.forks:
      torch.cuda.current_stream(self.device).wait_stream(self.stream)
    self.keep.clear()
    self.forks = 0


class _WrwQueue(object):

  def __init__(self, graph, direct, tensors):
    side = getattr(getattr(graph, 'store', None), 'wrw_side', None)
    self.side = side if (side is not None and side.armed and direct and not torch.cuda.is_current_stream_capturing()) else None
    self.graph, self.tensors, self.ctx = graph, tensors, None

  def __enter__(self):
    if self.side is None:
      return self.graph.scratch
    side = self.side
    side.stream.wait_stream(torch.cuda.current_stream(side.device))
    side.keep.append(self.tensors)
    side.forks += 1
    self.ctx = torch.cuda.stream(side.stream)
    self.ctx.__enter__()
    return side.scratch

  def __exit__(self, *exc):
    if self.ctx is not None:
      self.ctx.__exit__(*exc)
    return False


def _wrw_queue(graph, direct, *tensors):
  return _WrwQueue(graph, direct, tensors)


@contextlib.contextmanager
def wrw_side_armed(store: 'VarStore'):
  if not (WRW_SIDE and store is not None and getattr(store, 'device', None) is not None and torch.device(store.device).type == 'cuda'):
    yield
    return
  side = getattr(store, 'wrw_side', None)
  if side is None:
    side = store.wrw_side = WrwSide(store.device)
  side.armed = True
  try:
    yield
  finally:
    side.armed = False
    side.join()



def _nhwc(x: torch.Tensor) -> torch.Tensor:
  if x.dim() == 4:
    return x.contiguous(memory_format=torch.channels_last)
  return x.contiguous()


def _bn_fast_ok(C: int) -> bool:
  if C % 8:
    return False
  G = C // 8
  if G < 8:
    return 8 % G == 0
  return C % 64 == 0 and G <= 256 and 256 % G == 0


def _bn_blocks(rows: int, C: int) -> int:
  if _bn_fast_ok(C):
    cg = min(C // 8, 8)
    nslab = C // (cg * 8)
    row_lanes = 1024 // cg
    return int(max(1, min(256 // nslab, rows // (row_lanes * 2))))
  return int(min(256, max(1, rows // 64)))


class BnSums(object):
  __slots__ = ('x', 'scale_shift', 'mean_invstd', 'act', 'n_consumers', 'bwd_stats')

  def __init__(self):
    self.n_consumers = 0
    self.bwd_stats = None

  def sums_for(self, dq):
    bs = self.bwd_stats
    return bs[:2] if bs is not None and bs[2] == dq.data_ptr() else None

  def add_consumer(self, fuses: bool):
    self.n_consumers += 1 if fuses else 2

  @staticmethod
  def sums_buffer(G: int, C: int, device):
    return torch.empty((G, 2, C), dtype=torch.float32, device=device)

  def leave(self, partial, G: int, dx):
    self.bwd_stats = (partial, G, dx.data_ptr())


def _bn_enter(ctx, x, gamma, beta, layer, graph, training, slot, stats, rec=None, *more):
  x = _nhwc(x)
  C = gamma.numel()
  rows = x.numel() // C
  scale_shift, mean_invstd = _bn_scale_shift(x, gamma, beta, layer, graph, training, slot, stats)
  ctx.save_for_backward(x, scale_shift, mean_invstd, *more)
  ctx.bn = (layer.act, graph, rows, C, (gamma, beta), not training, rec)
  if rec is not None:
    rec.x, rec.scale_shift, rec.mean_invstd, rec.act = x, scale_shift, mean_invstd, layer.act
  return x, rows, C, scale_shift


def _bn_leave(ctx, dq, pre=None, **kw):
  x, scale_shift, mean_invstd = ctx.saved_tensors[:3]
  act, graph, rows, C, params, frozen, rec = ctx.bn
  if rec is not None:
    pre = rec.sums_for(dq)
  return _bn_backward(dq, x, scale_shift, mean_invstd, act, graph, rows, C, params=params, pre=pre, frozen=frozen, **kw)


class _BnActQuant(torch.autograd.Function):

  @staticmethod
  def forward(ctx, x, gamma, beta, layer, graph, training, slot, bits, stats=None, rec=None):
    x, rows, C, scale_shift = _bn_enter(ctx, x, gamma, beta, layer, graph, training, slot, stats, rec)
    quantize = bits is not None
    q = torch.empty_like(x)
# ... 1550 lines not shown
```

### pocketflow_amd/hip.py

```python
from __future__ import annotations

import ctypes
import os
from ctypes import c_float, c_int, c_int64, c_void_p

import numpy as np
import torch

_LIB_PATH = os.environ.get('PF_HIP_LIB') or os.path.join(os.path.dirname(os.path.abspath(__file__)), 'csrc', 'libpocketflow_hip.so')

PF_F32, PF_BF16 = 0, 1
PF_ACT_NONE, PF_ACT_RELU, PF_ACT_RELU6 = 0, 1, 2
PF_BUCKET_TENSOR, PF_BUCKET_CHANNEL, PF_BUCKET_SPLIT = 0, 1, 2
PF_CHUNK = 4096

SEG_DTYPE = np.dtype([('offset', '<i8'), ('len', '<i8'), ('RS', '<i4'), ('layout', '<i4'),
                      ('I', '<i4'), ('O', '<i4'), ('mode', '<i4'), ('bits', '<i4'),
                      ('bucket_size', '<i4'), ('n_bucket', '<i4'), ('slot_offset', '<i8'),
                      ('cb_offset', '<i8')])
BLOCK_DTYPE = np.dtype([('seg', '<i4'), ('chunk', '<i4'), ('row0', '<i4'), ('nrows', '<i4')])
assert SEG_DTYPE.itemsize == 64 and BLOCK_DTYPE.itemsize == 16

ACT_CODES = {None: PF_ACT_NONE, 'none': PF_ACT_NONE, 'Relu': PF_ACT_RELU, 'relu': PF_ACT_RELU,
             'Relu6': PF_ACT_RELU6, 'relu6': PF_ACT_RELU6}

SYMBOLS = [
    'pf_error_string', 'pf_version', 'pf_minmax_slots_init', 'pf_minmax_tensor', 'pf_minmax_decode',
    'pf_uq_apply', 'pf_act_grad', 'pf_seg_minmax', 'pf_seg_uq_apply', 'pf_seg_nuq_apply',
    'pf_seg_nuq_codebook_grad', 'pf_seg_normalize', 'pf_ws_bkup_merge_abs', 'pf_kth_largest_nonneg',
    'pf_ws_mask_apply', 'pf_count_nonzero', 'pf_cp_build_mask', 'pf_cp_mask_grad', 'pf_adam_flat',
    'pf_momentum_flat', 'pf_ce_distill_fwd_bwd', 'pf_bn_stats', 'pf_bn_finalize',
    'pf_bn_act_quant_apply', 'pf_bn_bwd_stats', 'pf_bn_bwd_finalize', 'pf_bn_bwd_apply', 'pf_bn_bwd_apply_add',
    'pf_bn_eval_scale_shift',
    'pf_conv1x1_stats_groups_k', 'pf_conv1x1_fwd', 'pf_conv1x1_bwd_data_bnstats', 'pf_conv1x1_wrw_splits',
    'pf_conv1x1_wrw', 'pf_conv2d_fwd', 'pf_conv2d_wrw_splits', 'pf_conv2d_wrw', 'pf_maxpool_fwd', 'pf_maxpool_bwd', 'pf_seg_transpose', 'pf_conv_stem_supported', 'pf_conv_stem_fwd', 'pf_conv_stem_wrw_slabs', 'pf_conv_stem_wrw',
    'pf_image_resize_bilinear', 'pf_depthwise_supported', 'pf_depthwise_groups', 'pf_depthwise_fwd', 'pf_depthwise_bwd_data',
    'pf_depthwise_wrw', 'pf_conv2d_stats_groups_geom', 'pf_tuning_reload',
    'pf_adam_flat_dev', 'pf_momentum_flat_dev', 'pf_set_floats',
    'pf_convg_fwd', 'pf_convg_bwd_data', 'pf_convg_small_splits', 'pf_convg_wrw_splits', 'pf_convg_wrw', 'pf_conv2d_bwd_data_strided',
    'pf_prox_groups', 'pf_prox_norms', 'pf_prox_apply', 'pf_im2col', 'pf_col2im',
    'pf_conv_stem3_supported', 'pf_conv_stem3_fwd', 'pf_conv_stem3_wrw_slabs', 'pf_conv_stem3_wrw',
    'pf_conv1x1_fwd_affine', 'pf_conv2d_fwd_affine', 'pf_conv2d_bwd_data_strided_stats_groups',
    'pf_conv2d_bwd_data_strided_bnstats',
    'pf_cpr_gather', 'pf_cpr_gram_ws', 'pf_cpr_gram', 'pf_cpr_ista', 'pf_cpr_lstsq_splits', 'pf_cpr_lstsq_step', 'pf_cpr_lstsq_resid',
    'pf_conv_gather_fwd',
    'pf_conv1x1_join_plan', 'pf_conv1x1_bwd_data_join',
    'pf_bn_act_quant_pool', 'pf_bn_bwd_stats_pooled', 'pf_bn_bwd_apply_pooled', 'pf_ce_distill_head', 'pf_ce_combine',
    'pf_bn_act_quant_codes', 'pf_conv_i8_supported', 'pf_conv_i8_fwd',
    'pf_dw_i8_supported', 'pf_dw_i8_fwd',
    'pf_bn_act_quant_static', 'pf_conv_i8_fwd_q', 'pf_dw_i8_fwd_q',
    'pf_bn_add_act_groups', 'pf_bn_add_act_fwd', 'pf_bn_add_act_bwd_gate', 'pf_bn_add_act_bwd_gate_add',
]


class HipLibraryMissing(RuntimeError):
  pass


def lib_path() -> str:
  return _LIB_PATH


def _load() -> ctypes.CDLL:
  if not os.path.exists(_LIB_PATH):
    raise HipLibraryMissing(
        'pocketflow_amd: %s not found -- build it with `python -c "import __graft_entry__ as g; '
        'g.build()"` or pocketflow_amd/csrc/build.sh.  There is no CPU fallback.' % _LIB_PATH)
  lib = ctypes.CDLL(_LIB_PATH)
  lib.pf_error_string.restype = ctypes.c_char_p
  lib.pf_error_string.argtypes = [c_int]
  lib.pf_version.restype = c_int
  for name in SYMBOLS:
    fn = getattr(lib, name)
    if name not in ('pf_error_string',):
      fn.restype = c_int
  lib.pf_cpr_gram_ws.restype = c_int64
  return lib


_lib = _load()


def _check(err: int, what: str) -> None:
  if err != 0:
    raise RuntimeError('%s failed: hipError %d (%s)' % (what, err, _lib.pf_error_string(err).decode()))


_raw_stream = getattr(torch._C, '_cuda_getCurrentRawStream', None)
_get_device = getattr(torch._C, '_cuda_getDevice', None)


def _stream() -> c_void_p:
  if _raw_stream is not None and _get_device is not None:
    return c_void_p(_raw_stream(_get_device()))
  return c_void_p(torch.cuda.current_stream().cuda_stream)


def _ptr(t) -> c_void_p:
  if t is None:
    return c_void_p(0)
  return c_void_p(t.data_ptr())


def dtype_code(t: torch.Tensor) -> int:
  if t.dtype == torch.float32:
    return PF_F32
  if t.dtype == torch.bfloat16:
    return PF_BF16
  raise TypeError('unsupported dtype %s (float32 / bfloat16 only)' % t.dtype)


def _dev(t: torch.Tensor) -> None:
  if not t.is_cuda:
    raise RuntimeError('pocketflow_amd kernels run on the GPU only (got a %s tensor)' % t.device)


def version() -> int:
  return int(_lib.pf_version())


def tuning_reload() -> None:
  _check(_lib.pf_tuning_reload(), 'pf_tuning_reload')



def minmax_slots_init(slots: torch.Tensor) -> None:
  _dev(slots)
  _check(_lib.pf_minmax_slots_init(_ptr(slots), c_int64(slots.numel() // 2), _stream()), 'pf_minmax_slots_init')


def minmax_tensor(x: torch.Tensor, slot: torch.Tensor, act=None) -> None:
  _dev(x)
  _check(_lib.pf_minmax_tensor(_ptr(x), c_int64(x.numel()), c_int(dtype_code(x)), c_int(ACT_CODES[act]),
                               _ptr(slot), _stream()), 'pf_minmax_tensor')


def minmax_decode(slots: torch.Tensor) -> torch.Tensor:
  n = slots.numel() // 2
  out = torch.empty((n, 2), dtype=torch.float32, device=slots.device)
  _check(_lib.pf_minmax_decode(_ptr(slots), c_int64(n), _ptr(out), _stream()), 'pf_minmax_decode')
  return out


def uq_apply(x: torch.Tensor, y: torch.Tensor, slot: torch.Tensor, bits: int, act=None) -> None:
  _dev(x)
  _check(_lib.pf_uq_apply(_ptr(x), _ptr(y), c_int64(x.numel()), c_int(dtype_code(x)), c_int(dtype_code(y)),
                          c_int(ACT_CODES[act]), _ptr(slot), c_int(int(bits)), _stream()), 'pf_uq_apply')


def act_grad(g: torch.Tensor, u: torch.Tensor, dx: torch.Tensor, act) -> None:
  _dev(g)
  assert g.dtype == u.dtype == dx.dtype
  _check(_lib.pf_act_grad(_ptr(g), _ptr(u), _ptr(dx), c_int64(g.numel()), c_int(dtype_code(g)),
                          c_int(ACT_CODES[act]), _stream()), 'pf_act_grad')



def seg_minmax(w_flat, segs, blocks, n_blocks, slots) -> None:
  _check(_lib.pf_seg_minmax(_ptr(w_flat), _ptr(segs), _ptr(blocks), c_int(n_blocks), _ptr(slots), _stream()),
         'pf_seg_minmax')


def seg_uq_apply(w_flat, qw_flat, segs, blocks, n_blocks, slots) -> None:
  _check(_lib.pf_seg_uq_apply(_ptr(w_flat), _ptr(qw_flat), c_int(dtype_code(qw_flat)), _ptr(segs), _ptr(blocks),
                              c_int(n_blocks), _ptr(slots), _stream()), 'pf_seg_uq_apply')


def seg_nuq_apply(w_flat, qw_flat, idx_flat, codebooks, segs, blocks, n_blocks, slots) -> None:
  _check(_lib.pf_seg_nuq_apply(_ptr(w_flat), _ptr(qw_flat), c_int(dtype_code(qw_flat)), _ptr(idx_flat),
                               _ptr(codebooks), _ptr(segs), _ptr(blocks), c_int(n_blocks), _ptr(slots),
                               _stream()), 'pf_seg_nuq_apply')


def seg_nuq_codebook_grad(g_flat, idx_flat, dcodebooks, acc_ws, segs, blocks, n_blocks, slots) -> None:
  assert acc_ws.dtype == torch.int64 and acc_ws.numel() >= dcodebooks.numel()
  _check(_lib.pf_seg_nuq_codebook_grad(_ptr(g_flat), c_int(dtype_code(g_flat)), _ptr(idx_flat), _ptr(dcodebooks),
                                       _ptr(acc_ws), c_int64(dcodebooks.numel()), _ptr(segs), _ptr(blocks),
                                       c_int(n_blocks), _ptr(slots), _stream()),
         'pf_seg_nuq_codebook_grad')


def seg_normalize(w_flat, xn_out, segs, seg_index, slots) -> None:
  _check(_lib.pf_seg_normalize(_ptr(w_flat), _ptr(xn_out), _ptr(segs), c_int(seg_index), _ptr(slots), _stream()),
         'pf_seg_normalize')



def ws_bkup_merge_abs(var, bkup, mask, abs_out) -> None:
  _check(_lib.pf_ws_bkup_merge_abs(_ptr(var), _ptr(bkup), _ptr(mask), _ptr(abs_out), c_int64(var.numel()),
                                   _stream()), 'pf_ws_bkup_merge_abs')


def kth_largest_nonneg(a, k_desc_index: int, out, workspace) -> None:
  _check(_lib.pf_kth_largest_nonneg(_ptr(a), c_int64(a.numel()), c_int64(int(k_desc_index)), _ptr(out),
                                    _ptr(workspace), _stream()), 'pf_kth_largest_nonneg')


def ws_mask_apply(var, bkup, mask, thr) -> None:
  _check(_lib.pf_ws_mask_apply(_ptr(var), _ptr(bkup), _ptr(mask), _ptr(thr), c_int64(var.numel()), _stream()),
         'pf_ws_mask_apply')


def count_nonzero(x, out_u64) -> None:
  _check(_lib.pf_count_nonzero(_ptr(x), c_int64(x.numel()), _ptr(out_u64), _stream()), 'pf_count_nonzero')


def cp_build_mask(mask, keep_in, keep_out, O: int, RS: int, I: int) -> None:
  _check(_lib.pf_cp_build_mask(_ptr(mask), _ptr(keep_in), _ptr(keep_out), c_int(O), c_int(RS), c_int(I),
                               _stream()), 'pf_cp_build_mask')


def cp_mask_grad(g, keep_in, keep_out, O: int, RS: int, I: int) -> None:
  _check(_lib.pf_cp_mask_grad(_ptr(g), _ptr(keep_in), _ptr(keep_out), c_int(O), c_int(RS), c_int(I), _stream()),
         'pf_cp_mask_grad')



def adam_flat(p, g, m, v, mask, n_decay: int, wd: float, g_scale: float, lr: float, beta1: float,
              beta2: float, eps: float, beta1_power: float, beta2_power: float) -> None:
  _check(_lib.pf_adam_flat(_ptr(p), _ptr(g), c_int(dtype_code(g)), _ptr(m), _ptr(v), _ptr(mask),
                           c_int64(p.numel()), c_int64(int(n_decay)), c_float(wd), c_float(g_scale), c_float(lr),
                           c_float(beta1), c_float(beta2), c_float(eps), c_float(beta1_power),
                           c_float(beta2_power), _stream()), 'pf_adam_flat')


def momentum_flat(p, g, acc, mask, n_decay: int, wd: float, g_scale: float, lr: float,
                  momentum: float) -> None:
  _check(_lib.pf_momentum_flat(_ptr(p), _ptr(g), c_int(dtype_code(g)), _ptr(acc), _ptr(mask), c_int64(p.numel()),
                               c_int64(int(n_decay)), c_float(wd), c_float(g_scale), c_float(lr),
                               c_float(momentum), _stream()), 'pf_momentum_flat')


def adam_flat_dev(p, g, m, v, mask, n_decay: int, wd: float, g_scale: float, hp, beta1: float, beta2: float,
                  eps: float) -> None:
  _check(_lib.pf_adam_flat_dev(_ptr(p), _ptr(g), c_int(dtype_code(g)), _ptr(m), _ptr(v), _ptr(mask),
                               c_int64(p.numel()), c_int64(int(n_decay)), c_float(wd), c_float(g_scale), _ptr(hp),
                               c_float(beta1), c_float(beta2), c_float(eps), _stream()), 'pf_adam_flat_dev')


def momentum_flat_dev(p, g, acc, mask, n_decay: int, wd: float, g_scale: float, hp, momentum: float) -> None:
  _check(_lib.pf_momentum_flat_dev(_ptr(p), _ptr(g), c_int(dtype_code(g)), _ptr(acc), _ptr(mask), c_int64(p.numel()),
                                   c_int64(int(n_decay)), c_float(wd), c_float(g_scale), _ptr(hp),
                                   c_float(momentum), _stream()), 'pf_momentum_flat_dev')


def set_floats(dst, a: float, b: float = 0.0, c: float = 0.0, d: float = 0.0) -> None:
  assert dst.dtype == torch.float32 and dst.numel() >= 4
  _check(_lib.pf_set_floats(_ptr(dst), c_float(a), c_float(b), c_float(c), c_float(d), _stream()), 'pf_set_floats')


def prox_groups(rows: int, I: int) -> int:
  return int(_lib.pf_prox_groups(c_int64(rows), c_int(I)))


def prox_norms(w, g, lr: float, rows: int, I: int, partial, norms) -> None:
  _dev(w)
  if w.dtype != torch.float32 or partial.numel() < prox_groups(rows, I) * I or norms.numel() < I:
    raise TypeError('prox_norms: float32 master kernel, workspace of prox_groups(rows, I) * I floats')
  _check(_lib.pf_prox_norms(_ptr(w), _ptr(g), c_int(dtype_code(g)), c_float(lr), c_int64(rows), c_int(I), _ptr(partial), _ptr(norms),
                            _stream()), 'pf_prox_norms')


def prox_apply(w, g, lr: float, rows: int, I: int, norms, thr) -> None:
  _dev(w)
  _check(_lib.pf_prox_apply(_ptr(w), _ptr(g), c_int(dtype_code(g)), c_float(lr), c_int64(rows), c_int(I), _ptr(norms), _ptr(thr),
                            _stream()), 'pf_prox_apply')



def _f32_dev(*ts) -> None:
  for t in ts:
    _dev(t)
    if t.dtype != torch.float32 or not t.is_contiguous():
      raise TypeError('pf_cpr: contiguous float32 tensors expected (got %s)' % t.dtype)


def _i32_dev(*ts) -> None:
  for t in ts:
    _dev(t)
    if t.dtype != torch.int32 or not t.is_contiguous():
      raise TypeError('pf_cpr: contiguous int32 tensors expected (got %s)' % t.dtype)


def cpr_gather(x, y, pos, kh: int, kw: int, stride: int, pad_t: int, pad_l: int, P, Y, row0: int) -> None:
  _dev(x)
  _dev(y)
  _i32_dev(pos)
  _f32_dev(P, Y)
  B, C, H, W = x.shape
  By, Co, OH, OW = y.shape
  crops = pos.shape[0]
  if By != B or not x.is_contiguous(memory_format=torch.channels_last) or not y.is_contiguous(memory_format=torch.channels_last):
    raise TypeError('cpr_gather: channels-last taps of one batch expected')
  if pos.numel() != 2 * crops or int(pos[:, 0].min()) < 0 or int(pos[:, 0].max()) >= OH or int(pos[:, 1].min()) < 0 or int(pos[:, 1].max()) >= OW:
    raise ValueError('cpr_gather: positions outside the %d x %d output' % (OH, OW))
  rows = row0 + crops * B
  if P.numel() < rows * kh * kw * C or Y.numel() < rows * Co:
    raise ValueError('cpr_gather: P / Y hold fewer than %d rows' % rows)
  _check(_lib.pf_cpr_gather(_ptr(x), c_int(dtype_code(x)), _ptr(y), c_int(dtype_code(y)), _ptr(pos), c_int(crops), c_int(B), c_int(H), c_int(W),
                            c_int(C), c_int(OH), c_int(OW), c_int(Co), c_int(kh), c_int(kw), c_int(stride), c_int(pad_t), c_int(pad_l), _ptr(P),
                            _ptr(Y), c_int64(row0), _stream()), 'pf_cpr_gather')


def cpr_gram_ws(C: int) -> int:
  return int(_lib.pf_cpr_gram_ws(c_int(C)))


def cpr_gram(P, Y, idx, kk: int, C: int, Co: int, w_krsc, ws, xtx, xty) -> None:
  _f32_dev(P, Y, w_krsc, xtx, xty)
  _i32_dev(idx)
  _dev(ws)
  rows = P.numel() // (kk * C)
  if ws.dtype != torch.float64 or ws.numel() < cpr_gram_ws(C) or w_krsc.numel() != Co * kk * C or xtx.numel() < C * C or xty.numel() < C:
    raise ValueError('cpr_gram: buffer sizes')
  if idx.numel() and (int(idx.min()) < 0 or int(idx.max()) >= rows or Y.numel() < rows * Co):
    raise ValueError('cpr_gram: row indices outside the %d sampled rows' % rows)
  _check(_lib.pf_cpr_gram(_ptr(P), _ptr(Y), _ptr(idx), c_int64(idx.numel()), c_int(kk), c_int(C), c_int(Co), _ptr(w_krsc), _ptr(ws),
                          c_int64(ws.numel()), _ptr(xtx), _ptr(xty), _stream()), 'pf_cpr_gram')


def cpr_ista(A, b, m0, m_ws, mask, gamma: float, lr: float, iters: int, nnz) -> None:
  C = b.numel()
  _f32_dev(A, b, m0, m_ws, mask)
  _i32_dev(nnz)
  if A.numel() != C * C or m0.numel() != C or m_ws.numel() < 2 * C or mask.numel() != C:
    raise ValueError('cpr_ista: buffer sizes')
  _check(_lib.pf_cpr_ista(_ptr(A), _ptr(b), _ptr(m0), _ptr(m_ws), _ptr(mask), c_int(C), c_float(gamma), c_float(lr), c_int(iters), _ptr(nnz),
                          _stream()), 'pf_cpr_ista')


def cpr_lstsq_splits(N: int, Kp: int, Co: int) -> int:
  return int(_lib.pf_cpr_lstsq_splits(c_int64(N), c_int(Kp), c_int(Co)))


def _lstsq_check(P, kidx, Y, R, W, N, Co):
  _f32_dev(P, Y, R, W)
  _i32_dev(kidx)
  K = W.numel() // Co
  if P.numel() < N * K or Y.numel() < N * Co or R.numel() < N * Co or W.numel() != K * Co:
    raise ValueError('cpr_lstsq: buffer sizes')
  if kidx.numel() and (int(kidx.min()) < 0 or int(kidx.max()) >= K):
    raise ValueError('cpr_lstsq: kept rows outside the kernel')
  return K


def cpr_lstsq_step(P, kidx, pos, Y, R, W, m, v, part, N: int, Co: int, wd: float, lr_t: float, beta1: float, beta2: float, c1: float,
                   c2: float, eps: float) -> None:
  K = _lstsq_check(P, kidx, Y, R, W, N, Co)
  _f32_dev(m, v, part)
  _i32_dev(pos)
  Kp = kidx.numel()
  if pos.numel() != K or m.numel() != K * Co or v.numel() != K * Co or part.numel() < cpr_lstsq_splits(N, Kp, Co) * Kp * Co:
    raise ValueError('cpr_lstsq_step: buffer sizes')
  _check(_lib.pf_cpr_lstsq_step(_ptr(P), c_int(K), _ptr(kidx), _ptr(pos), c_int(Kp), _ptr(Y), _ptr(R), c_int64(N), c_int(Co), _ptr(W), _ptr(m),
                                _ptr(v), _ptr(part), c_float(wd), c_float(lr_t), c_float(beta1), c_float(beta2), c_float(c1), c_float(c2),
                                c_float(eps), _stream()), 'pf_cpr_lstsq_step')


def cpr_lstsq_resid(P, kidx, W, Y, R, N: int, Co: int) -> None:
  K = _lstsq_check(P, kidx, Y, R, W, N, Co)
  _check(_lib.pf_cpr_lstsq_resid(_ptr(P), c_int(K), _ptr(kidx), c_int(kidx.numel()), _ptr(W), _ptr(Y), _ptr(R), c_int64(N), c_int(Co),
                                 _stream()), 'pf_cpr_lstsq_resid')



def ce_distill_fwd_bwd(z_s, labels, z_t, tempr: float, loss_w: float, losses, dz_s, row_ws) -> None:
  B, C = z_s.shape
  _check(_lib.pf_ce_distill_fwd_bwd(_ptr(z_s), c_int(dtype_code(z_s)), _ptr(labels), _ptr(z_t),
                                    c_int(dtype_code(z_t) if z_t is not None else 0), c_int(B), c_int(C),
                                    c_float(tempr), c_float(loss_w), _ptr(losses), _ptr(dz_s),
                                    c_int(dtype_code(dz_s)), _ptr(row_ws), _stream()), 'pf_ce_distill_fwd_bwd')


def ce_distill_head(z_s, labels, z_t, tempr: float, loss_w: float, losses, dz_hard, dz_soft, row_ws) -> None:
  B, C = z_s.shape
  _check(_lib.pf_ce_distill_head(_ptr(z_s), c_int(dtype_code(z_s)), _ptr(labels), _ptr(z_t),
                                 c_int(dtype_code(z_t) if z_t is not None else 0), c_int(B), c_int(C),
                                 c_float(tempr), c_float(loss_w), _ptr(losses), _ptr(dz_hard), _ptr(dz_soft),
                                 c_int(dtype_code(dz_hard)), _ptr(row_ws), _stream()), 'pf_ce_distill_head')


def ce_combine(dz_hard, dz_soft, g0, g1, dz) -> None:
  _check(_lib.pf_ce_combine(_ptr(dz_hard), _ptr(dz_soft), _ptr(g0), _ptr(g1), _ptr(dz), c_int(dtype_code(dz)),
                            c_int64(dz.numel()), _stream()), 'pf_ce_combine')



def bn_stats(x, rows: int, C: int, partial, n_blocks: int) -> None:
  _check(_lib.pf_bn_stats(_ptr(x), c_int(dtype_code(x)), c_int64(rows), c_int(C), _ptr(partial), c_int(n_blocks),
                          _stream()), 'pf_bn_stats')


def bn_finalize(partial, n_blocks, rows, C, x, gamma, beta, moving_mean, moving_var, momentum, eps,
                training: bool, act, scale_shift, mean_invstd, slot) -> None:
  _check(_lib.pf_bn_finalize(_ptr(partial), c_int(n_blocks), c_int64(rows), c_int(C), _ptr(x),
                             c_int(dtype_code(x)), _ptr(gamma), _ptr(beta), _ptr(moving_mean), _ptr(moving_var),
                             c_float(momentum), c_float(eps), c_int(1 if training else 0), c_int(ACT_CODES[act]),
                             _ptr(scale_shift), _ptr(mean_invstd), _ptr(slot), _stream()), 'pf_bn_finalize')


def bn_act_quant_apply(x, q, rows, C, scale_shift, act, slot, bits: int, quantize: bool) -> None:
  _check(_lib.pf_bn_act_quant_apply(_ptr(x), _ptr(q), c_int(dtype_code(x)), c_int64(rows), c_int(C),
                                    _ptr(scale_shift), c_int(ACT_CODES[act]), _ptr(slot), c_int(int(bits)),
                                    c_int(1 if quantize else 0), _stream()), 'pf_bn_act_quant_apply')


def bn_act_quant_pool(x, pooled, rows, C, hw: int, scale_shift, act, slot, bits: int, quantize: bool) -> None:
  _check(_lib.pf_bn_act_quant_pool(_ptr(x), _ptr(pooled), c_int(dtype_code(x)), c_int64(rows), c_int(C),
                                   _ptr(scale_shift), c_int(ACT_CODES[act]), _ptr(slot), c_int(int(bits)),
                                   c_int(1 if quantize else 0), c_int(hw), _stream()), 'pf_bn_act_quant_pool')


def bn_bwd_stats_pooled(g, x, rows, C, hw: int, scale_shift, mean_invstd, act, partial, n_blocks) -> None:
  _check(_lib.pf_bn_bwd_stats_pooled(_ptr(g), _ptr(x), c_int(dtype_code(x)), c_int64(rows), c_int(C), c_int(hw),
                                     _ptr(scale_shift), _ptr(mean_invstd), c_int(ACT_CODES[act]), _ptr(partial),
                                     c_int(n_blocks), _stream()), 'pf_bn_bwd_stats_pooled')


def bn_bwd_apply_pooled(g, x, dx, rows, C, hw: int, scale_shift, mean_invstd, dgamma, dbeta, act) -> None:
  _check(_lib.pf_bn_bwd_apply_pooled(_ptr(g), _ptr(x), _ptr(dx), c_int(dtype_code(x)), c_int64(rows), c_int(C),
                                     c_int(hw), _ptr(scale_shift), _ptr(mean_invstd), _ptr(dgamma), _ptr(dbeta),
                                     c_int(ACT_CODES[act]), _stream()), 'pf_bn_bwd_apply_pooled')


def bn_bwd_stats(dq, x, rows, C, scale_shift, mean_invstd, act, partial, n_blocks) -> None:
  _check(_lib.pf_bn_bwd_stats(_ptr(dq), _ptr(x), c_int(dtype_code(x)), c_int64(rows), c_int(C), _ptr(scale_shift),
                              _ptr(mean_invstd), c_int(ACT_CODES[act]), _ptr(partial), c_int(n_blocks),
                              _stream()), 'pf_bn_bwd_stats')


def bn_bwd_finalize(partial, n_blocks, C, dgamma, dbeta) -> None:
  _check(_lib.pf_bn_bwd_finalize(_ptr(partial), c_int(n_blocks), c_int(C), _ptr(dgamma), _ptr(dbeta), _stream()),
         'pf_bn_bwd_finalize')


def bn_bwd_apply(dq, x, dx, rows, C, scale_shift, mean_invstd, dgamma, dbeta, act, addend=None) -> None:
  _check(_lib.pf_bn_bwd_apply_add(_ptr(dq), _ptr(x), _ptr(addend), _ptr(dx), c_int(dtype_code(x)), c_int64(rows),
                                  c_int(C), _ptr(scale_shift), _ptr(mean_invstd), _ptr(dgamma), _ptr(dbeta),
                                  c_int(ACT_CODES[act]), _stream()), 'pf_bn_bwd_apply_add')


def bn_eval_scale_shift(gamma, beta, moving_mean, moving_var, eps: float, scale_shift) -> None:
  _check(_lib.pf_bn_eval_scale_shift(_ptr(gamma), _ptr(beta), _ptr(moving_mean), _ptr(moving_var), c_float(eps),
                                     c_int(gamma.numel()), _ptr(scale_shift), _stream()), 'pf_bn_eval_scale_shift')


def bn_add_act_groups(rows: int, C: int) -> int:
  return int(_lib.pf_bn_add_act_groups(c_int64(rows), c_int(C)))


def bn_add_act_fwd(x, r, u, rows, C, scale_shift, act, slot=None) -> None:
  _check(_lib.pf_bn_add_act_fwd(_ptr(x), _ptr(r), _ptr(u), c_int(dtype_code(x)), c_int64(rows), c_int(C), _ptr(scale_shift),
                                c_int(ACT_CODES[act]), _ptr(slot), _stream()), 'pf_bn_add_act_fwd')


def bn_add_act_bwd_gate(dq, x, r, g, rows, C, scale_shift, mean_invstd, act, partial, addend=None) -> None:
  if addend is None:
    _check(_lib.pf_bn_add_act_bwd_gate(_ptr(dq), _ptr(x), _ptr(r), _ptr(g), c_int(dtype_code(x)), c_int64(rows), c_int(C),
                                       _ptr(scale_shift), _ptr(mean_invstd), c_int(ACT_CODES[act]), _ptr(partial), _stream()),
           'pf_bn_add_act_bwd_gate')
    return
  _check(_lib.pf_bn_add_act_bwd_gate_add(_ptr(dq), _ptr(addend), _ptr(x), _ptr(r), _ptr(g), c_int(dtype_code(x)), c_int64(rows),
                                         c_int(C), _ptr(scale_shift), _ptr(mean_invstd), c_int(ACT_CODES[act]), _ptr(partial),
                                         _stream()), 'pf_bn_add_act_bwd_gate_add')



def conv1x1_stats_groups(M: int, N: int, K: int, prologue: bool = False) -> int:
  return int(_lib.pf_conv1x1_stats_groups_k(c_int(M), c_int(N), c_int(K), c_int(1 if prologue else 0)))


def conv1x1_wrw_splits(M: int, N: int, K: int) -> int:
  return int(_lib.pf_conv1x1_wrw_splits(c_int(M), c_int(N), c_int(K)))


def conv1x1_fwd(X, W, Y, M: int, N: int, K: int, R=None, scale_shift=None, act=None, slot=None, bits: int = 8,
                partial=None, geom=None, ymap: bool = False, out_scale_shift=None, out_act=None) -> None:
  _dev(X)
  Ho, Wo, H, Wd, stride = geom if geom is not None else (0, 0, 0, 0, 1)
  if out_scale_shift is not None:
    if R is not None or partial is not None or slot is not None or ymap:
      raise ValueError('the folded output pass takes no residual, statistics, quantiser or row map')
    _check(_lib.pf_conv1x1_fwd_affine(_ptr(X), _ptr(W), _ptr(Y), _ptr(scale_shift), c_int(ACT_CODES[act]), _ptr(out_scale_shift),
                                      c_int(ACT_CODES[out_act]), c_int(M), c_int(N), c_int(K), c_int(Ho), c_int(Wo), c_int(H),
                                      c_int(Wd), c_int(stride), _stream()), 'pf_conv1x1_fwd_affine')
    return
  _check(_lib.pf_conv1x1_fwd(_ptr(X), _ptr(W), _ptr(Y), _ptr(R), _ptr(scale_shift), c_int(ACT_CODES[act]),
                             _ptr(slot), c_int(int(bits)), _ptr(partial), c_int(M), c_int(N), c_int(K), c_int(Ho),
                             c_int(Wo), c_int(H), c_int(Wd), c_int(stride), c_int(1 if ymap else 0), _stream()),
         'pf_conv1x1_fwd')


def conv1x1_wrw(dY, X, dW, workspace, M: int, N: int, K: int, scale_shift=None, act=None, slot=None,
                bits: int = 8, geom=None) -> None:
  _dev(X)
  Ho, Wo, H, Wd, stride = geom if geom is not None else (0, 0, 0, 0, 1)
  _check(_lib.pf_conv1x1_wrw(_ptr(dY), _ptr(X), _ptr(dW), c_int(dtype_code(dW)), _ptr(workspace), _ptr(scale_shift),
                             c_int(ACT_CODES[act]), _ptr(slot), c_int(int(bits)), c_int(M), c_int(N), c_int(K),
                             c_int(Ho), c_int(Wo), c_int(H), c_int(Wd), c_int(stride), _stream()), 'pf_conv1x1_wrw')


def conv1x1_bwd_data_bnstats(dY, Wt, dQ, bn_x, bn_scale_shift, bn_mean_invstd, bn_act, partial, M: int, N: int,
                             K: int) -> None:
  _dev(dY)
  _check(_lib.pf_conv1x1_bwd_data_bnstats(_ptr(dY), _ptr(Wt), _ptr(dQ), _ptr(bn_x), _ptr(bn_scale_shift),
                                          _ptr(bn_mean_invstd), c_int(ACT_CODES[bn_act]), _ptr(partial), c_int(M),
                                          c_int(N), c_int(K), _stream()), 'pf_conv1x1_bwd_data_bnstats')


def conv1x1_join_plan(M: int, N: int, K: int, with_stats: bool = False) -> int:
  return int(_lib.pf_conv1x1_join_plan(c_int(M), c_int(N), c_int(K), c_int(1 if with_stats else 0)))


def conv1x1_bwd_data_join(dY, Wt, dQ, R, M: int, N: int, K: int, rgeom=None, bn_x=None, bn_scale_shift=None,
                          bn_mean_invstd=None, bn_act=None, partial=None) -> None:
  _dev(dY)
  Ho, Wo, H, Wd, stride = rgeom if rgeom is not None else (0, 0, 0, 0, 1)
  _check(_lib.pf_conv1x1_bwd_data_join(_ptr(dY), _ptr(Wt), _ptr(dQ), _ptr(R), c_int(Ho), c_int(Wo), c_int(H), c_int(Wd),
                                       c_int(stride), _ptr(bn_x), _ptr(bn_scale_shift), _ptr(bn_mean_invstd),
                                       c_int(ACT_CODES[bn_act]), _ptr(partial), c_int(M), c_int(N), c_int(K), _stream()),
         'pf_conv1x1_bwd_data_join')



_zero_page = {}


def zero_page(device):
  key = str(device)
  z = _zero_page.get(key)
  if z is None:
    z = _zero_page[key] = torch.zeros(256, dtype=torch.bfloat16, device=device)
  return z


def conv2d_stats_groups(M: int, N: int, geom=None) -> int:
  if geom is None:
    raise ValueError('conv2d_stats_groups: pass geom = (imgs, H, Wd, C, N, th, tw, stride, pad_h, pad_w, Ho, Wo) of the pf_conv2d_fwd call')
  return int(_lib.pf_conv2d_stats_groups_geom(*[c_int(int(v)) for v in geom]))


def conv2d_fwd(X, W, Y, imgs: int, H: int, Wd: int, C: int, N: int, th: int, tw: int, stride: int, pad_h: int,
               pad_w: int, Ho: int, Wo: int, R=None, partial=None, bn_x=None, bn_scale_shift=None,
               bn_mean_invstd=None, bn_act=None, out_scale_shift=None, out_act=None) -> None:
  _dev(X)
  if out_scale_shift is not None:
# ... 367 lines not shown
```

### pocketflow_amd/optim.py

```python
from __future__ import annotations

from typing import List, Optional

import numpy as np
import torch
import torch.distributed as dist

from pocketflow_amd import hip
from pocketflow_amd.graph import VarStore


class FlatOptimizer(object):
  def __init__(self, store: VarStore, kind: str = 'adam', momentum: float = 0.9, beta1: float = 0.9,
               beta2: float = 0.999, epsilon: float = 1e-8, weight_decay: float = 0.0):
    if kind not in ('adam', 'momentum'):
      raise ValueError('unknown optimizer kind: ' + kind)
    self.store, self.kind = store, kind
    self.momentum, self.beta1, self.beta2, self.epsilon = momentum, beta1, beta2, epsilon
    self.weight_decay = weight_decay
    dev = store.device
    self.slots_w = [torch.zeros_like(store.w_master) for _ in range(2 if kind == 'adam' else 1)]
    self.slots_o = [torch.zeros_like(store.o_master) for _ in range(2 if kind == 'adam' else 1)]
    self.beta1_power = np.float32(beta1)
    self.beta2_power = np.float32(beta2)
    self.w_mask: Optional[torch.Tensor] = None
    self.o_mask: Optional[torch.Tensor] = None
    self.g_scale = 1.0
    self.w_grad_src: Optional[torch.Tensor] = None
    self.o_grad_src: Optional[torch.Tensor] = None
    self.hp: Optional[torch.Tensor] = None
    self.hyper_external = False

  def enable_device_hyper(self) -> None:
    if self.hp is None:
      self.hp = torch.zeros(4, dtype=torch.float32, device=self.store.device)

  def feed_hyper(self, lrn_rate: float) -> None:
    one = np.float32(1.0)
    alpha_t = 0.0
    if self.kind == 'adam':
      alpha_t = float(np.float32(np.float32(lrn_rate) * np.sqrt(one - np.float32(self.beta2_power))) / (one - np.float32(self.beta1_power)))
      self.beta1_power = np.float32(self.beta1_power * np.float32(self.beta1))
      self.beta2_power = np.float32(self.beta2_power * np.float32(self.beta2))
    hip.set_floats(self.hp, alpha_t, float(lrn_rate))

  def state_tensors(self) -> List[torch.Tensor]:
    return self.slots_w + self.slots_o

  def reset_slots(self) -> None:
    for t in self.state_tensors():
      t.zero_()
    self.beta1_power = np.float32(self.beta1)
    self.beta2_power = np.float32(self.beta2)

  def backward(self, loss: torch.Tensor) -> None:
    from pocketflow_amd import graph as G
    with G.wrw_side_armed(self.store):
      loss.backward()

  def compute_gradients(self) -> None:
    self.g_scale = 1.0
    self.w_grad_src = self.o_grad_src = None

  def apply_gradients(self, lrn_rate: float) -> None:
    st = self.store
    wd = float(self.weight_decay)
    w_grad = self.w_grad_src if self.w_grad_src is not None else st.w_grad
    o_grad = self.o_grad_src if self.o_grad_src is not None else st.o_grad
    if self.hp is not None:
      if not self.hyper_external:
        self.feed_hyper(lrn_rate)
      if self.kind == 'adam':
        if st.w_size:
          hip.adam_flat_dev(st.w_master, w_grad, self.slots_w[0], self.slots_w[1], self.w_mask, st.w_decay, wd, self.g_scale,
                            self.hp, self.beta1, self.beta2, self.epsilon)
        if st.o_size:
          hip.adam_flat_dev(st.o_master, o_grad, self.slots_o[0], self.slots_o[1], self.o_mask, st.o_decay, wd, self.g_scale,
                            self.hp, self.beta1, self.beta2, self.epsilon)
      else:
        if st.w_size:
          hip.momentum_flat_dev(st.w_master, w_grad, self.slots_w[0], self.w_mask, st.w_decay, wd, self.g_scale, self.hp,
                                self.momentum)
        if st.o_size:
          hip.momentum_flat_dev(st.o_master, o_grad, self.slots_o[0], self.o_mask, st.o_decay, wd, self.g_scale, self.hp,
                                self.momentum)
      st.w_t_fresh = False
      st.zero_grad()
      return
    if self.kind == 'adam':
      b1p, b2p = float(self.beta1_power), float(self.beta2_power)
      if st.w_size:
        hip.adam_flat(st.w_master, w_grad, self.slots_w[0], self.slots_w[1], self.w_mask, st.w_decay, wd,
                      self.g_scale, lrn_rate, self.beta1, self.beta2, self.epsilon, b1p, b2p)
      if st.o_size:
        hip.adam_flat(st.o_master, o_grad, self.slots_o[0], self.slots_o[1], self.o_mask, st.o_decay, wd,
                      self.g_scale, lrn_rate, self.beta1, self.beta2, self.epsilon, b1p, b2p)
      self.beta1_power = np.float32(self.beta1_power * np.float32(self.beta1))
      self.beta2_power = np.float32(self.beta2_power * np.float32(self.beta2))
    else:
      if st.w_size:
        hip.momentum_flat(st.w_master, w_grad, self.slots_w[0], self.w_mask, st.w_decay, wd, self.g_scale,
                          lrn_rate, self.momentum)
      if st.o_size:
        hip.momentum_flat(st.o_master, o_grad, self.slots_o[0], self.o_mask, st.o_decay, wd, self.g_scale,
                          lrn_rate, self.momentum)
    st.w_t_fresh = False
    st.zero_grad()


class GradReducer(object):

  def __init__(self, store: VarStore, bucket_elems: int = 8 << 20, reduce_dtype: Optional[torch.dtype] = torch.float32,
               overlap: bool = True):
    self.store = store
    self.overlap = overlap
    self.reduce_dtype = reduce_dtype
    self.buckets = []
    self.var_bucket = {}
    self._build_buckets(bucket_elems)
    self._stage_w: Optional[torch.Tensor] = None
    self._stage_o: Optional[torch.Tensor] = None
    self._reset_cycle()
    self.armed = False
    store.grad_hook = self._on_grad
    self.n_overlapped = 0
    self.recorder = None

  def _build_buckets(self, bucket_elems: int) -> None:
    ws = sorted([v for v in self.store.vars if v.group == 'W' and v.trainable], key=lambda v: v.offset)
    lo, cnt = 0, 0
    for i, v in enumerate(ws):
      self.var_bucket[v.name] = len(self.buckets)
      cnt += 1
      end = v.offset + v.numel
      last = i == len(ws) - 1
      if last:
        end = self.store.w_size
      if end - lo >= bucket_elems or last:
        self.buckets.append([lo, end, cnt])
        lo, cnt = end, 0

  def _reset_cycle(self) -> None:
    self.pending = [b[2] for b in self.buckets]
    self.seen = set()
    self.launched = [False] * len(self.buckets)
    self.handles = []
    self.dirty = False

  def _active(self) -> bool:
    return dist.is_initialized() and dist.get_world_size() > 1

  def _stage(self, which: str) -> torch.Tensor:
    st = self.store
    src = st.w_grad if which == 'w' else st.o_grad
    dt = self.reduce_dtype or src.dtype
    buf = self._stage_w if which == 'w' else self._stage_o
    if buf is None or buf.dtype != dt:
      buf = torch.empty(src.numel(), dtype=dt, device=src.device)
      if which == 'w':
        self._stage_w = buf
      else:
        self._stage_o = buf
    return buf

  def _stage_bucket(self, b: int):
    lo, hi, _ = self.buckets[b]
    piece = self._stage('w')[lo:hi]
    side = getattr(self.store, 'wrw_side', None)
    if side is not None and side.forks and self.store.w_grad.is_cuda:
      cur = torch.cuda.current_stream(self.store.w_grad.device)
      if cur != side.stream:
        cur.wait_stream(side.stream)
    piece.copy_(self.store.w_grad[lo:hi])
    self.launched[b] = True
    return lambda: self.handles.append(dist.all_reduce(piece, op=dist.ReduceOp.SUM, async_op=True))

  def _launch(self, b: int) -> None:
    self._stage_bucket(b)()

  def _recording(self) -> bool:
    return self.recorder is not None and getattr(self.recorder, 'capturing', False)

  def arm(self) -> None:
    for h in self.handles:
      h.wait()
    self._reset_cycle()
    self.armed = True

  def disarm(self) -> None:
    self.armed = False

  def _on_grad(self, var) -> None:
    if not (self.overlap and self._active()) or var.group != 'W' or self._recording():
      return
    if not self.armed:
      if any(self.launched):
        self.dirty = True
      return
    b = self.var_bucket.get(var.name)
    if b is None:
      return
    if var.name in self.seen:
      return
    self.seen.add(var.name)
    self.pending[b] -= 1
    if self.pending[b] == 0 and not self.launched[b]:
      self._launch(b)
      self.n_overlapped += 1

  def finish(self):
    st = self.store
    self.armed = False
    if not self._active():
      self._reset_cycle()
      return st.w_grad, st.o_grad, 1.0
    n_over = sum(self.launched)
    if self.dirty:
      for h in self.handles:
        h.wait()
      self.handles = []
      self.launched = [False] * len(self.buckets)
      n_over = 0
    calls = []
    if st.w_size:
      calls = [self._stage_bucket(b) for b in range(len(self.buckets)) if not self.launched[b]]
    w_src = self._stage('w') if st.w_size else st.w_grad
    o_src = st.o_grad
    if st.o_size:
      o_src = self._stage('o')
      o_src.copy_(st.o_grad)
    o_piece = o_src if st.o_size else None

    def exchange():
      for call in calls:
        call()
      if o_piece is not None:
        self.handles.append(dist.all_reduce(o_piece, op=dist.ReduceOp.SUM, async_op=True))
      for h in self.handles:
        h.wait()
      self.handles = []
    if self.recorder is not None:
      self.recorder.cut(exchange)
    else:
      exchange()
    self._reset_cycle()
    self.n_overlapped = n_over
    return w_src, o_src, 1.0 / dist.get_world_size()


def grad_reducer_of(store: VarStore) -> GradReducer:
  r = getattr(store, 'reducer', None)
  if r is None:
    import os
    from pocketflow_amd.flags import FLAGS
    rd = {'float32': torch.float32, 'compute': None}[FLAGS.allreduce_dtype if 'allreduce_dtype' in FLAGS else 'float32']
    r = GradReducer(store, bucket_elems=int(os.environ.get('PF_ALLREDUCE_BUCKET', 8 << 20)), reduce_dtype=rd,
                    overlap=os.environ.get('PF_OVERLAP_ALLREDUCE', '1') != '0')
    store.reducer = r
  return r


class DistributedFlatOptimizer(object):

  _OWN = ('opt', 'reducer')

  def __init__(self, optimizer: FlatOptimizer):
    object.__setattr__(self, 'opt', optimizer)
    object.__setattr__(self, 'reducer', grad_reducer_of(optimizer.store))

  def __getattr__(self, name):
    return getattr(self.opt, name)

  def __setattr__(self, name, value):
    if name in DistributedFlatOptimizer._OWN:
      object.__setattr__(self, name, value)
    else:
      setattr(self.opt, name, value)

  def backward(self, loss: torch.Tensor) -> None:
    from pocketflow_amd import graph as G
    self.reducer.arm()
    try:
      with G.wrw_side_armed(self.opt.store):
        loss.backward()
    finally:
      self.reducer.disarm()

  def compute_gradients(self) -> None:
    w_src, o_src, scale = self.reducer.finish()
    self.opt.w_grad_src, self.opt.o_grad_src = w_src, o_src
    self.opt.g_scale = scale

  def apply_gradients(self, lrn_rate: float) -> None:
    self.opt.apply_gradients(lrn_rate)
```

Before: 11460.

## Fuse gradient zeroing into optimizer kernels and rework maxpool and transpose kernels

Adds optimizer kernel variants that write zeros back to the gradient buffer right after reading it. This lets the separate zero_grad memset be skipped whenever the store owns the gradient buffer. The maxpool forward kernel is also restructured: neighbor offsets are precomputed once and reused across the batch via grid.y, there is a fast max path that skips masking for unclipped windows, and an optional index output. The segment transpose gets an alignment flag so it can use vector paths. Together these mix unrelated kernel changes and add template variants and code complexity.

Result: no change. 11440 (-0.2%).

```diff
diff --git a/include/pocketflow_hip.h b/include/pocketflow_hip.h
--- a/include/pocketflow_hip.h
+++ b/include/pocketflow_hip.h
@@ -82,6 +82,18 @@
                          int64_t n, int64_t n_decay, float wd, float g_scale, const float* hp,
                          float momentum, void* stream);
 int pf_set_floats(float* dst, float a, float b, float c, float d, void* stream);
+int pf_adam_flat_zero(float* p, void* g, int g_dtype, float* m, float* v, const float* mask,
+                      int64_t n, int64_t n_decay, float wd, float g_scale, float lr, float beta1,
+                      float beta2, float eps, float beta1_power, float beta2_power, void* stream);
+int pf_momentum_flat_zero(float* p, void* g, int g_dtype, float* acc, const float* mask,
+                          int64_t n, int64_t n_decay, float wd, float g_scale, float lr, float momentum,
+                          void* stream);
+int pf_adam_flat_zero_dev(float* p, void* g, int g_dtype, float* m, float* v, const float* mask,
+                          int64_t n, int64_t n_decay, float wd, float g_scale, const float* hp, float beta1,
+                          float beta2, float eps, void* stream);
+int pf_momentum_flat_zero_dev(float* p, void* g, int g_dtype, float* acc, const float* mask,
+                              int64_t n, int64_t n_decay, float wd, float g_scale, const float* hp,
+                              float momentum, void* stream);
 
 int pf_ce_distill_fwd_bwd(const void* z_s, int zs_dtype, const float* labels, const void* z_t,
                           int zt_dtype, int B, int C, float tempr, float loss_w, float* losses,
diff --git a/pocketflow_amd/csrc/pf_optim.hip b/pocketflow_amd/csrc/pf_optim.hip
--- a/pocketflow_amd/csrc/pf_optim.hip
+++ b/pocketflow_amd/csrc/pf_optim.hip
@@ -18,8 +18,12 @@
   return ge * mask;
 }
 
-template <typename TG, bool MASK>
-__global__ __launch_bounds__(PF_THREADS) void k_adam_flat(float* __restrict__ p, const TG* __restrict__ g,
+template <typename TG> __device__ __forceinline__ void zero4g(TG* p);
+template <> __device__ __forceinline__ void zero4g<float>(float* p) { *reinterpret_cast<float4*>(p) = make_float4(0.f, 0.f, 0.f, 0.f); }
+template <> __device__ __forceinline__ void zero4g<bf16_t>(bf16_t* p) { *reinterpret_cast<uint2*>(p) = make_uint2(0u, 0u); }
+
+template <typename TG, bool MASK, bool ZERO>
+__global__ __launch_bounds__(PF_THREADS) void k_adam_flat(float* __restrict__ p, TG* __restrict__ g,
                                                           float* __restrict__ m, float* __restrict__ v,
                                                           const float* __restrict__ mask, int64_t n,
                                                           int64_t n_decay, float wd, float g_scale,
@@ -47,11 +51,13 @@
     *reinterpret_cast<float4*>(p + e) = make_float4(pa[0], pa[1], pa[2], pa[3]);
     *reinterpret_cast<float4*>(m + e) = make_float4(ma[0], ma[1], ma[2], ma[3]);
     *reinterpret_cast<float4*>(v + e) = make_float4(va[0], va[1], va[2], va[3]);
+    if (ZERO) zero4g<TG>(g + e);
   }
   if (blockIdx.x == 0) {
     for (int64_t e = (nv << 2) + threadIdx.x; e < n; e += PF_THREADS) {
       const float mk = MASK ? mask[e] : 1.0f;
       const float ge = eff_grad(load_one<TG>(g + e), p[e], mk, e < n_decay, wd, g_scale);
+      if (ZERO) g[e] = (TG)0;
       const float mn = m[e] + (ge - m[e]) * omb1;
       const float vn = v[e] + (ge * ge - v[e]) * omb2;
       m[e] = mn; v[e] = vn;
@@ -60,7 +66,7 @@
   }
 }
 
-static int adam_launch(float* p, const void* g, int g_dtype, float* m, float* v,
+static int adam_launch(float* p, void* g, bool zero, int g_dtype, float* m, float* v,
                        const float* mask, int64_t n, int64_t n_decay, float wd, float g_scale,
                        float lr, float beta1, float beta2, float eps, float beta1_power,
                        float beta2_power, const float* hp, void* stream) {
@@ -72,10 +78,12 @@
   const float omb1 = 1.0f - beta1, omb2 = 1.0f - beta2;
   hipStream_t st = (hipStream_t)stream;
   const int grid = pf_grid_for(n, PF_THREADS * 4);
-#define PF_AD(TG, MK) k_adam_flat<TG, MK><<<grid, PF_THREADS, 0, st>>>(p, (const TG*)g, m, v, mask, n, n_decay, wd, g_scale, alpha_t, omb1, omb2, eps, hp)
-  if (g_dtype == PF_F32) { if (mask) PF_AD(float, true); else PF_AD(float, false); }
-  else if (g_dtype == PF_BF16) { if (mask) PF_AD(bf16_t, true); else PF_AD(bf16_t, false); }
+#define PF_AD(TG, MK, ZR) k_adam_flat<TG, MK, ZR><<<grid, PF_THREADS, 0, st>>>(p, (TG*)g, m, v, mask, n, n_decay, wd, g_scale, alpha_t, omb1, omb2, eps, hp)
+#define PF_AD2(TG, MK) do { if (zero) PF_AD(TG, MK, true); else PF_AD(TG, MK, false); } while (0)
+  if (g_dtype == PF_F32) { if (mask) PF_AD2(float, true); else PF_AD2(float, false); }
+  else if (g_dtype == PF_BF16) { if (mask) PF_AD2(bf16_t, true); else PF_AD2(bf16_t, false); }
   else return (int)hipErrorInvalidValue;
+#undef PF_AD2
 #undef PF_AD
   PF_LAUNCH_CHECK();
   return 0;
@@ -85,19 +93,35 @@
                             const float* mask, int64_t n, int64_t n_decay, float wd, float g_scale,
                             float lr, float beta1, float beta2, float eps, float beta1_power,
                             float beta2_power, void* stream) {
-  return adam_launch(p, g, g_dtype, m, v, mask, n, n_decay, wd, g_scale, lr, beta1, beta2, eps, beta1_power, beta2_power, nullptr,
-                     stream);
+  return adam_launch(p, const_cast<void*>(g), false, g_dtype, m, v, mask, n, n_decay, wd, g_scale, lr, beta1, beta2, eps, beta1_power,
+                     beta2_power, nullptr, stream);
+}
+
+extern "C" int pf_adam_flat_zero(float* p, void* g, int g_dtype, float* m, float* v,
+                                 const float* mask, int64_t n, int64_t n_decay, float wd, float g_scale,
+                                 float lr, float beta1, float beta2, float eps, float beta1_power,
+                                 float beta2_power, void* stream) {
+  return adam_launch(p, g, true, g_dtype, m, v, mask, n, n_decay, wd, g_scale, lr, beta1, beta2, eps, beta1_power, beta2_power,
+                     nullptr, stream);
 }
 
 extern "C" int pf_adam_flat_dev(float* p, const void* g, int g_dtype, float* m, float* v,
                                 const float* mask, int64_t n, int64_t n_decay, float wd, float g_scale,
                                 const float* hp, float beta1, float beta2, float eps, void* stream) {
   if (hp == nullptr) return (int)hipErrorInvalidValue;
-  return adam_launch(p, g, g_dtype, m, v, mask, n, n_decay, wd, g_scale, 0.f, beta1, beta2, eps, 0.5f, 0.5f, hp, stream);
-}
-
-template <typename TG, bool MASK>
-__global__ __launch_bounds__(PF_THREADS) void k_momentum_flat(float* __restrict__ p, const TG* __restrict__ g,
+  return adam_launch(p, const_cast<void*>(g), false, g_dtype, m, v, mask, n, n_decay, wd, g_scale, 0.f, beta1, beta2, eps, 0.5f, 0.5f,
+                     hp, stream);
+}
+
+extern "C" int pf_adam_flat_zero_dev(float* p, void* g, int g_dtype, float* m, float* v,
+                                     const float* mask, int64_t n, int64_t n_decay, float wd, float g_scale,
+                                     const float* hp, float beta1, float beta2, float eps, void* stream) {
+  if (hp == nullptr) return (int)hipErrorInvalidValue;
+  return adam_launch(p, g, true, g_dtype, m, v, mask, n, n_decay, wd, g_scale, 0.f, beta1, beta2, eps, 0.5f, 0.5f, hp, stream);
+}
+
+template <typename TG, bool MASK, bool ZERO>
+__global__ __launch_bounds__(PF_THREADS) void k_momentum_flat(float* __restrict__ p, TG* __restrict__ g,
                                                               float* __restrict__ acc,
                                                               const float* __restrict__ mask, int64_t n,
                                                               int64_t n_decay, float wd, float g_scale,
@@ -121,11 +145,13 @@
     }
     *reinterpret_cast<float4*>(p + e) = make_float4(pa[0], pa[1], pa[2], pa[3]);
     *reinterpret_cast<float4*>(acc + e) = make_float4(ac[0], ac[1], ac[2], ac[3]);
+    if (ZERO) zero4g<TG>(g + e);
   }
   if (blockIdx.x == 0) {
     for (int64_t e = (nv << 2) + threadIdx.x; e < n; e += PF_THREADS) {
       const float mk = MASK ? mask[e] : 1.0f;
       const float ge = eff_grad(load_one<TG>(g + e), p[e], mk, e < n_decay, wd, g_scale);
+      if (ZERO) g[e] = (TG)0;
       const float a = mu * acc[e] + ge;
       acc[e] = a;
       p[e] = p[e] - lr * a;
@@ -133,7 +159,7 @@
   }
 }
 
-static int momentum_launch(float* p, const void* g, int g_dtype, float* acc, const float* mask,
+static int momentum_launch(float* p, void* g, bool zero, int g_dtype, float* acc, const float* mask,
                            int64_t n, int64_t n_decay, float wd, float g_scale, float lr,
                            float momentum, const float* hp, void* stream) {
   if (n <= 0) return 0;
@@ -141,10 +167,12 @@
     return (int)hipErrorInvalidValue;
   hipStream_t st = (hipStream_t)stream;
   const int grid = pf_grid_for(n, PF_THREADS * 4);
-#define PF_MO(TG, MK) k_momentum_flat<TG, MK><<<grid, PF_THREADS, 0, st>>>(p, (const TG*)g, acc, mask, n, n_decay, wd, g_scale, lr, momentum, hp)
-  if (g_dtype == PF_F32) { if (mask) PF_MO(float, true); else PF_MO(float, false); }
-  else if (g_dtype == PF_BF16) { if (mask) PF_MO(bf16_t, true); else PF_MO(bf16_t, false); }
+#define PF_MO(TG, MK, ZR) k_momentum_flat<TG, MK, ZR><<<grid, PF_THREADS, 0, st>>>(p, (TG*)g, acc, mask, n, n_decay, wd, g_scale, lr, momentum, hp)
+#define PF_MO2(TG, MK) do { if (zero) PF_MO(TG, MK, true); else PF_MO(TG, MK, false); } while (0)
+  if (g_dtype == PF_F32) { if (mask) PF_MO2(float, true); else PF_MO2(float, false); }
+  else if (g_dtype == PF_BF16) { if (mask) PF_MO2(bf16_t, true); else PF_MO2(bf16_t, false); }
   else return (int)hipErrorInvalidValue;
+#undef PF_MO2
 #undef PF_MO
   PF_LAUNCH_CHECK();
   return 0;
@@ -153,14 +181,27 @@
 extern "C" int pf_momentum_flat(float* p, const void* g, int g_dtype, float* acc, const float* mask,
                                 int64_t n, int64_t n_decay, float wd, float g_scale, float lr,
                                 float momentum, void* stream) {
-  return momentum_launch(p, g, g_dtype, acc, mask, n, n_decay, wd, g_scale, lr, momentum, nullptr, stream);
+  return momentum_launch(p, const_cast<void*>(g), false, g_dtype, acc, mask, n, n_decay, wd, g_scale, lr, momentum, nullptr, stream);
+}
+
+extern "C" int pf_momentum_flat_zero(float* p, void* g, int g_dtype, float* acc, const float* mask,
+                                     int64_t n, int64_t n_decay, float wd, float g_scale, float lr,
+                                     float momentum, void* stream) {
+  return momentum_launch(p, g, true, g_dtype, acc, mask, n, n_decay, wd, g_scale, lr, momentum, nullptr, stream);
 }
 
 extern "C" int pf_momentum_flat_dev(float* p, const void* g, int g_dtype, float* acc, const float* mask,
                                     int64_t n, int64_t n_decay, float wd, float g_scale, const float* hp,
                                     float momentum, void* stream) {
   if (hp == nullptr) return (int)hipErrorInvalidValue;
-  return momentum_launch(p, g, g_dtype, acc, mask, n, n_decay, wd, g_scale, 0.f, momentum, hp, stream);
+  return momentum_launch(p, const_cast<void*>(g), false, g_dtype, acc, mask, n, n_decay, wd, g_scale, 0.f, momentum, hp, stream);
+}
+
+extern "C" int pf_momentum_flat_zero_dev(float* p, void* g, int g_dtype, float* acc, const float* mask,
+                                         int64_t n, int64_t n_decay, float wd, float g_scale, const float* hp,
+                                         float momentum, void* stream) {
+  if (hp == nullptr) return (int)hipErrorInvalidValue;
+  return momentum_launch(p, g, true, g_dtype, acc, mask, n, n_decay, wd, g_scale, 0.f, momentum, hp, stream);
 }
 
 __global__ void k_set_floats(float* __restrict__ dst, float a, float b, float c, float d) {
diff --git a/pocketflow_amd/csrc/pf_pool.hip b/pocketflow_amd/csrc/pf_pool.hip
--- a/pocketflow_amd/csrc/pf_pool.hip
+++ b/pocketflow_amd/csrc/pf_pool.hip
@@ -80,55 +80,123 @@
   }
 }
 
-template <typename T>
+
+template <typename T> __device__ __forceinline__ void store8_exact(T* __restrict__ p, const float* in);
+template <> __device__ __forceinline__ void store8_exact<float>(float* __restrict__ p, const float* in) { store8<float>(p, in); }
+template <> __device__ __forceinline__ void store8_exact<bf16_t>(bf16_t* __restrict__ p, const float* in) {
+  uint4 v;
+  v.x = (__float_as_uint(in[0]) >> 16) | (__float_as_uint(in[1]) & 0xFFFF0000u);
+  v.y = (__float_as_uint(in[2]) >> 16) | (__float_as_uint(in[3]) & 0xFFFF0000u);
+  v.z = (__float_as_uint(in[4]) >> 16) | (__float_as_uint(in[5]) & 0xFFFF0000u);
+  v.w = (__float_as_uint(in[6]) >> 16) | (__float_as_uint(in[7]) & 0xFFFF0000u);
+  *reinterpret_cast<uint4*>(p) = v;
+}
+
+template <typename T, bool IDX>
 __global__ __launch_bounds__(PF_THREADS) void k_maxpool3s2_fwd(const T* __restrict__ x, T* __restrict__ y,
                                                                uint8_t* __restrict__ idx, int B, int H, int W, int C,
                                                                int pad_h, int pad_w, int Ho, int Wo) {
   const int CV = C >> 3;
-  const int total = B * Ho * Wo * CV;
-  for (int64_t e64 = (int64_t)blockIdx.x * PF_THREADS + threadIdx.x; e64 < total; e64 += (int64_t)gridDim.x * PF_THREADS) {
-    const int e = (int)e64;
-    const int cv = e % CV;
-    int p = e / CV;
-    const int wo = p % Wo; p /= Wo;
-    const int ho = p % Ho;
-    const int b = p / Ho;
-    const int h0 = ho * 2 - pad_h, w0 = wo * 2 - pad_w;
+  const int i = blockIdx.x * PF_THREADS + threadIdx.x;
+  if (i >= Ho * Wo * CV) return;
+  const int cv = i % CV;
+  const int p = i / CV;
+  const int wo = p % Wo, ho = p / Wo;
+  const int h0 = ho * 2 - pad_h, w0 = wo * 2 - pad_w;
+  const bool clipped = h0 < 0 || h0 + 2 >= H || w0 < 0 || w0 + 2 >= W;
+  int off[9];
+#pragma unroll
+  for (int r = 0; r < 3; ++r) {
+    const int hi = h0 + r;
+    const int hc = hi < 0 ? 0 : (hi >= H ? H - 1 : hi);
+#pragma unroll
+    for (int s = 0; s < 3; ++s) {
+      const int wi = w0 + s;
+      const int wc = wi < 0 ? 0 : (wi >= W ? W - 1 : wi);
+      off[r * 3 + s] = (hc * W + wc) * C + (cv << 3);
+    }
+  }
+  const int64_t in_img = (int64_t)H * W * C, out_img = (int64_t)Ho * Wo * C;
+  const int64_t o_in = (int64_t)p * C + (cv << 3);
+  for (int b = blockIdx.y; b < B; b += gridDim.y) {
+    const T* __restrict__ xb = x + b * in_img;
     float v[9][8];
 #pragma unroll
-    for (int r = 0; r < 3; ++r)
-#pragma unroll
-      for (int s = 0; s < 3; ++s) {
-        const int hi = h0 + r, wi = w0 + s;
-        const int hc = hi < 0 ? 0 : (hi >= H ? H - 1 : hi), wc = wi < 0 ? 0 : (wi >= W ? W - 1 : wi);
-        load8<T>(x + (((int64_t)b * H + hc) * W + wc) * C + (cv << 3), v[r * 3 + s]);
-      }
-#pragma unroll
-    for (int r = 0; r < 3; ++r)
-#pragma unroll
-      for (int s = 0; s < 3; ++s) {
-        const bool ok = (unsigned)(h0 + r) < (unsigned)H && (unsigned)(w0 + s) < (unsigned)W;
-#pragma unroll
-        for (int j = 0; j < 8; ++j) v[r * 3 + s][j] = ok ? v[r * 3 + s][j] : -INFINITY;
-      }
+    for (int t = 0; t < 9; ++t) load8<T>(xb + off[t], v[t]);
+    if (clipped) {
+#pragma unroll
+      for (int r = 0; r < 3; ++r)
+#pragma unroll
+        for (int s = 0; s < 3; ++s) {
+          const bool ok = (unsigned)(h0 + r) < (unsigned)H && (unsigned)(w0 + s) < (unsigned)W;
+#pragma unroll
+          for (int j = 0; j < 8; ++j) v[r * 3 + s][j] = ok ? v[r * 3 + s][j] : -INFINITY;
+        }
+    }
     float best[8];
     int arg[8];
-#pragma unroll
-    for (int j = 0; j < 8; ++j) { best[j] = -INFINITY; arg[j] = 0; }
-#pragma unroll
-    for (int t = 0; t < 9; ++t)
-#pragma unroll
-      for (int j = 0; j < 8; ++j)
-        if (v[t][j] > best[j] || v[t][j] != v[t][j]) { best[j] = v[t][j]; arg[j] = t; }
-    const int64_t o = (((int64_t)b * Ho + ho) * Wo + wo) * C + (cv << 3);
-    store8<T>(y + o, best);
-    if (idx != nullptr) {
+    bool any_nan = false, any_zero = false;
+#pragma unroll
+    for (int j = 0; j < 8; ++j) {
+      float m = v[0][j];
+#pragma unroll
+      for (int t = 1; t < 9; ++t) m = __builtin_elementwise_maximum(m, v[t][j]);
+      best[j] = m;
+      any_nan |= m != m;
+      any_zero |= m == 0.f;
+    }
+    if (!any_nan) {
+      if (IDX) {
+#pragma unroll
+        for (int j = 0; j < 8; ++j) {
+          arg[j] = 8;
+#pragma unroll
+          for (int t = 7; t >= 0; --t) arg[j] = v[t][j] == best[j] ? t : arg[j];
+        }
+      }
+      if (any_zero) {
+#pragma unroll
+        for (int j = 0; j < 8; ++j) {
+          float b0 = v[8][j];
+#pragma unroll
+          for (int t = 7; t >= 0; --t) b0 = v[t][j] == best[j] ? v[t][j] : b0;
+          best[j] = b0;
+        }
+      }
+    } else {
+#pragma unroll
+      for (int j = 0; j < 8; ++j) { best[j] = -INFINITY; arg[j] = 0; }
+#pragma unroll
+      for (int t = 0; t < 9; ++t)
+#pragma unroll
+        for (int j = 0; j < 8; ++j)
+          if (v[t][j] > best[j] || v[t][j] != v[t][j]) { best[j] = v[t][j]; arg[j] = t; }
+    }
+    const int64_t o = b * out_img + o_in;
+    if (!any_nan) store8_exact<T>(y + o, best);
+    else store8<T>(y + o, best);
+    if (IDX) {
       uint2 pk;
       pk.x = (uint32_t)arg[0] | ((uint32_t)arg[1] << 8) | ((uint32_t)arg[2] << 16) | ((uint32_t)arg[3] << 24);
       pk.y = (uint32_t)arg[4] | ((uint32_t)arg[5] << 8) | ((uint32_t)arg[6] << 16) | ((uint32_t)arg[7] << 24);
       *reinterpret_cast<uint2*>(idx + o) = pk;
     }
   }
+}
+
+template <typename T> __device__ __forceinline__ void store8_finite(T* __restrict__ p, const float* in);
+template <> __device__ __forceinline__ void store8_finite<float>(float* __restrict__ p, const float* in) { store8<float>(p, in); }
+__device__ __forceinline__ uint32_t rne_bf16_bits(float f) {
+  const uint32_t u = __float_as_uint(f);
+  return u + 0x7FFFu + ((u >> 16) & 1u);
+}
+template <> __device__ __forceinline__ void store8_finite<bf16_t>(bf16_t* __restrict__ p, const float* in) {
+  uint4 v;
+  v.x = (rne_bf16_bits(in[0]) >> 16) | (rne_bf16_bits(in[1]) & 0xFFFF0000u);
+  v.y = (rne_bf16_bits(in[2]) >> 16) | (rne_bf16_bits(in[3]) & 0xFFFF0000u);
+  v.z = (rne_bf16_bits(in[4]) >> 16) | (rne_bf16_bits(in[5]) & 0xFFFF0000u);
+  v.w = (rne_bf16_bits(in[6]) >> 16) | (rne_bf16_bits(in[7]) & 0xFFFF0000u);
+  *reinterpret_cast<uint4*>(p) = v;
 }
 
 template <typename T>
@@ -136,39 +204,48 @@
                                                                T* __restrict__ dx, int B, int H, int W, int C, int pad_h,
                                                                int pad_w, int Ho, int Wo, int Ha, int Wb) {
   const int CV = C >> 3;
-  const int total = B * Ha * Wb * CV;
-  for (int64_t e64 = (int64_t)blockIdx.x * PF_THREADS + threadIdx.x; e64 < total; e64 += (int64_t)gridDim.x * PF_THREADS) {
-    const int e = (int)e64;
-    const int cv = e % CV;
-    int p = e / CV;
-    const int bb = p % Wb; p /= Wb;
-    const int a = p % Ha;
-    const int b = p / Ha;
+  const int e = blockIdx.x * PF_THREADS + threadIdx.x;
+  if (e >= Ha * Wb * CV) return;
+  const int cv = e % CV;
+  const int p = e / CV;
+  const int bb = p % Wb, a = p / Wb;
+  int off_w[2][2], off_p[2][2];
+  bool ok_w[2][2], ok_p[2][2];
+#pragma unroll
+  for (int i = 0; i < 2; ++i)
+#pragma unroll
+    for (int k = 0; k < 2; ++k) {
+      const int ho = a - i, wo = bb - k;
+      ok_w[i][k] = (unsigned)ho < (unsigned)Ho && (unsigned)wo < (unsigned)Wo;
+      const int hoc = ho < 0 ? 0 : (ho >= Ho ? Ho - 1 : ho), woc = wo < 0 ? 0 : (wo >= Wo ? Wo - 1 : wo);
+      off_w[i][k] = (hoc * Wo + woc) * C + (cv << 3);
+      const int hi = 2 * a + i - pad_h, wi = 2 * bb + k - pad_w;
+      ok_p[i][k] = (unsigned)hi < (unsigned)H && (unsigned)wi < (unsigned)W;
+      off_p[i][k] = ok_p[i][k] ? (hi * W + wi) * C + (cv << 3) : 0;
+    }
+  const int64_t in_img = (int64_t)H * W * C, out_img = (int64_t)Ho * Wo * C;
+  for (int b = blockIdx.y; b < B; b += gridDim.y) {
+    const T* __restrict__ dyb = dy + b * out_img;
+    const uint8_t* __restrict__ idxb = idx + b * out_img;
+    T* __restrict__ dxb = dx + b * in_img;
     float d[2][2][8];
     uint2 pk[2][2];
 #pragma unroll
     for (int i = 0; i < 2; ++i)
 #pragma unroll
       for (int k = 0; k < 2; ++k) {
-        const int ho = a - i, wo = bb - k;
-        const bool ok = (unsigned)ho < (unsigned)Ho && (unsigned)wo < (unsigned)Wo;
-        const int hoc = ho < 0 ? 0 : (ho >= Ho ? Ho - 1 : ho), woc = wo < 0 ? 0 : (wo >= Wo ? Wo - 1 : wo);
-        const int64_t o = (((int64_t)b * Ho + hoc) * Wo + woc) * C + (cv << 3);
-        const uint2 pki = *reinterpret_cast<const uint2*>(idx + o);
-        load8<T>(dy + o, d[i][k]);
-        pk[i][k] = ok ? pki : make_uint2(0xFFFFFFFFu, 0xFFFFFFFFu);
-      }
-#pragma unroll
-    for (int du = 0; du < 2; ++du) {
-      const int hi = 2 * a + du - pad_h;
-      if ((unsigned)hi >= (unsigned)H) continue;
+        const uint2 pki = *reinterpret_cast<const uint2*>(idxb + off_w[i][k]);
+        load8<T>(dyb + off_w[i][k], d[i][k]);
+        pk[i][k] = ok_w[i][k] ? pki : make_uint2(0xFFFFFFFFu, 0xFFFFFFFFu);
+      }
+    float g[2][2][8];
+    bool any_nan = false;
+#pragma unroll
+    for (int du = 0; du < 2; ++du)
 #pragma unroll
       for (int dv = 0; dv < 2; ++dv) {
-        const int wi = 2 * bb + dv - pad_w;
-        if ((unsigned)wi >= (unsigned)W) continue;
-        float g[8];
-#pragma unroll
-        for (int j = 0; j < 8; ++j) g[j] = 0.f;
+#pragma unroll
+        for (int j = 0; j < 8; ++j) g[du][dv][j] = 0.f;
 #pragma unroll
         for (int i = 0; i < 2; ++i) {
           const int r = du + 2 * i;
@@ -181,20 +258,28 @@
 #pragma unroll
             for (int j = 0; j < 8; ++j) {
               const uint32_t t = ((j < 4 ? pk[i][k].x : pk[i][k].y) >> ((j & 3) * 8)) & 0xFFu;
-              if (t == want) g[j] += d[i][k][j];
+              g[du][dv][j] = g[du][dv][j] + (t == want ? d[i][k][j] : 0.f);
             }
           }
         }
-        store8<T>(dx + (((int64_t)b * H + hi) * W + wi) * C + (cv << 3), g);
-      }
-    }
+#pragma unroll
+        for (int j = 0; j < 8; ++j) any_nan |= g[du][dv][j] != g[du][dv][j];
+      }
+#pragma unroll
+    for (int du = 0; du < 2; ++du)
+#pragma unroll
+      for (int dv = 0; dv < 2; ++dv)
+        if (ok_p[du][dv]) {
+          if (!any_nan) store8_finite<T>(dxb + off_p[du][dv], g[du][dv]);
+          else store8<T>(dxb + off_p[du][dv], g[du][dv]);
+        }
   }
 }
 
 static bool pool3s2_ok(int B, int H, int W, int C, int k, int stride, int pad_h, int pad_w, int Ho, int Wo) {
   if (pf_tuning().pool3s2 == 0) return false;
   return k == 3 && stride == 2 && pad_h >= 0 && pad_h <= 1 && pad_w >= 0 && pad_w <= 1 &&
-         (int64_t)B * H * W * (C / 8) < (1ll << 31);
+         (int64_t)B * H * W * (C / 8) < (1ll << 31) && (int64_t)H * W * C < (1ll << 31);
 }
 
 extern "C" int pf_maxpool_fwd(const void* x, void* y, void* idx, int dtype, int B, int H, int W, int C, int k, int stride,
@@ -206,10 +291,17 @@
   const int grid = pf_grid_for(total, PF_THREADS);
   hipStream_t st = (hipStream_t)stream;
   if (pool3s2_ok(B, H, W, C, k, stride, pad_h, pad_w, Ho, Wo) && (dtype == PF_F32 || dtype == PF_BF16)) {
-    if (dtype == PF_F32)
-      k_maxpool3s2_fwd<float><<<grid, PF_THREADS, 0, st>>>((const float*)x, (float*)y, (uint8_t*)idx, B, H, W, C, pad_h, pad_w, Ho, Wo);
-    else
-      k_maxpool3s2_fwd<bf16_t><<<grid, PF_THREADS, 0, st>>>((const bf16_t*)x, (bf16_t*)y, (uint8_t*)idx, B, H, W, C, pad_h, pad_w, Ho, Wo);
+    const int gx = (int)(((int64_t)Ho * Wo * (C / 8) + PF_THREADS - 1) / PF_THREADS);
+    int gy = (2 * PF_MAX_GRID + gx - 1) / gx;
+    gy = gy > B ? B : gy;
+    const dim3 g3(gx, gy);
+    pf_with_bool(idx != nullptr, [&](auto I) {
+      constexpr bool IDX = decltype(I)::value;
+      if (dtype == PF_F32)
+        k_maxpool3s2_fwd<float, IDX><<<g3, PF_THREADS, 0, st>>>((const float*)x, (float*)y, (uint8_t*)idx, B, H, W, C, pad_h, pad_w, Ho, Wo);
+      else
+        k_maxpool3s2_fwd<bf16_t, IDX><<<g3, PF_THREADS, 0, st>>>((const bf16_t*)x, (bf16_t*)y, (uint8_t*)idx, B, H, W, C, pad_h, pad_w, Ho, Wo);
+    });
     PF_LAUNCH_CHECK();
     return 0;
   }
@@ -234,7 +326,10 @@
   hipStream_t st = (hipStream_t)stream;
   if (pool3s2_ok(B, H, W, C, k, stride, pad_h, pad_w, Ho, Wo) && (dtype == PF_F32 || dtype == PF_BF16)) {
     const int Ha = (H + pad_h + 1) / 2, Wb = (W + pad_w + 1) / 2;
-    const int g2 = pf_grid_for((int64_t)B * Ha * Wb * (C / 8), PF_THREADS);
+    const int gx = (int)(((int64_t)Ha * Wb * (C / 8) + PF_THREADS - 1) / PF_THREADS);
+    int gy = (2 * PF_MAX_GRID + gx - 1) / gx;
+    gy = gy > B ? B : gy;
+    const dim3 g2(gx, gy);
     if (dtype == PF_F32)
       k_maxpool3s2_bwd<float><<<g2, PF_THREADS, 0, st>>>((const float*)dy, (const uint8_t*)idx, (float*)dx, B, H, W, C, pad_h, pad_w, Ho, Wo, Ha, Wb);
     else
diff --git a/pocketflow_amd/csrc/pf_quant.hip b/pocketflow_amd/csrc/pf_quant.hip
--- a/pocketflow_amd/csrc/pf_quant.hip
+++ b/pocketflow_amd/csrc/pf_quant.hip
@@ -200,6 +200,14 @@
   return rs * (uint32_t)sg.I + i;
 }
 
+#define PF_MM_GROUP 8
+#define PF_MM_UNROLL 8
+
+__device__ __forceinline__ void mm_acc4(float& mn, float& mx, const float4 v) {
+  mn = fminf(fminf(mn, v.x), fminf(v.y, fminf(v.z, v.w)));
+  mx = fmaxf(fmaxf(mx, v.x), fmaxf(v.y, fmaxf(v.z, v.w)));
+}
+
 __global__ __launch_bounds__(PF_THREADS) void k_seg_minmax(const float* __restrict__ w,
                                                            const PfSeg* __restrict__ segs,
                                                            const PfBlock* __restrict__ blocks,
@@ -272,18 +280,28 @@
     return;
   }
 
+  const int n_chunks = (int)((sg.len + PF_CHUNK - 1) / PF_CHUNK);
+  const int group = b.chunk / PF_MM_GROUP, first = group * PF_MM_GROUP;
+  const int in_group = min(PF_MM_GROUP, n_chunks - first);
+  if (b.chunk - first != group % in_group) return;
+  const int64_t g0 = (int64_t)first * PF_CHUNK;
+  const int64_t e1 = min(sg.len, g0 + (int64_t)PF_MM_GROUP * PF_CHUNK);
+  const int64_t nv = (e1 - g0) >> 2;
+  const float4* __restrict__ v4 = reinterpret_cast<const float4*>(base + g0);
   float mn = INFINITY, mx = -INFINITY;
-#pragma unroll
-  for (int it = 0; it < 4; ++it) {
-    const int64_t e = e0 + it * 1024 + threadIdx.x * 4;
-    if (e + 3 < sg.len) {
-      float4 v = *reinterpret_cast<const float4*>(base + e);
-      mn = fminf(fminf(mn, v.x), fminf(v.y, fminf(v.z, v.w)));
-      mx = fmaxf(fmaxf(mx, v.x), fmaxf(v.y, fmaxf(v.z, v.w)));
-    } else {
-      for (int j = 0; j < 4; ++j)
-        if (e + j < sg.len) { float v = base[e + j]; mn = fminf(mn, v); mx = fmaxf(mx, v); }
-    }
+  int64_t i = threadIdx.x;
+  for (; i + (PF_MM_UNROLL - 1) * PF_THREADS < nv; i += PF_MM_UNROLL * PF_THREADS) {
+    float4 q[PF_MM_UNROLL];
+#pragma unroll
+    for (int k = 0; k < PF_MM_UNROLL; ++k) q[k] = v4[i + k * PF_THREADS];
+#pragma unroll
+    for (int k = 0; k < PF_MM_UNROLL; ++k) mm_acc4(mn, mx, q[k]);
+  }
+  for (; i < nv; i += PF_THREADS) mm_acc4(mn, mx, v4[i]);
+  for (int64_t e = g0 + (nv << 2) + threadIdx.x; e < e1; e += PF_THREADS) {
+    const float v = base[e];
+    mn = fminf(mn, v);
+    mx = fmaxf(mx, v);
   }
   block_minmax(mn, mx, lds);
   if (threadIdx.x == 0 && mn <= mx) {
diff --git a/pocketflow_amd/csrc/pf_transpose.hip b/pocketflow_amd/csrc/pf_transpose.hip
--- a/pocketflow_amd/csrc/pf_transpose.hip
+++ b/pocketflow_amd/csrc/pf_transpose.hip
@@ -9,11 +9,44 @@
   int32_t pad0, pad1;
 };
 
+#define PF_TR_PITCH 33
+__device__ __forceinline__ void transpose_tile_vec(const bf16_t* __restrict__ s, bf16_t* __restrict__ d, int src_ld, int dst_ld,
+                                                   uint32_t* __restrict__ tl) {
+  const int v = threadIdx.x & 7, row = threadIdx.x >> 3;
+#pragma unroll
+  for (int h = 0; h < 2; ++h) {
+    const int o = row + 32 * h;
+    const uint4 q = *reinterpret_cast<const uint4*>(s + (int64_t)o * src_ld + (v << 3));
+    uint32_t* __restrict__ w = tl + o * PF_TR_PITCH + (v << 2);
+    w[0] = q.x; w[1] = q.y; w[2] = q.z; w[3] = q.w;
+  }
+  __syncthreads();
+  const bf16_t* __restrict__ te = reinterpret_cast<const bf16_t*>(tl);
+#pragma unroll
+  for (int h = 0; h < 2; ++h) {
+    const int i = row + 32 * h;
+    uint32_t e[8];
+#pragma unroll
+    for (int j = 0; j < 8; ++j) e[j] = te[((v << 3) + j) * (2 * PF_TR_PITCH) + i];
+    uint4 q;
+    q.x = e[0] | (e[1] << 16); q.y = e[2] | (e[3] << 16); q.z = e[4] | (e[5] << 16); q.w = e[6] | (e[7] << 16);
+    *reinterpret_cast<uint4*>(d + (int64_t)i * dst_ld + (v << 3)) = q;
+  }
+}
+
 template <typename T>
 __global__ __launch_bounds__(PF_THREADS) void k_seg_transpose(const T* __restrict__ src, T* __restrict__ dst,
-                                                              const PfTile* __restrict__ tiles) {
+                                                              const PfTile* __restrict__ tiles, int vec_ok) {
   __shared__ T tile[64][65];
   const PfTile t = tiles[blockIdx.x];
+  if constexpr (std::is_same<T, bf16_t>::value) {
+    __shared__ uint32_t tl[64 * PF_TR_PITCH];
+    if (vec_ok && t.o0 + 64 <= t.O && t.i0 + 64 <= t.I && (((t.src_off | t.dst_off) | (int64_t)(t.src_ld | t.dst_ld | t.o0 | t.i0)) & 7) == 0) {
+      transpose_tile_vec(src + t.src_off + (int64_t)t.o0 * t.src_ld + t.i0, dst + t.dst_off + (int64_t)t.i0 * t.dst_ld + t.o0, t.src_ld,
+                         t.dst_ld, tl);
+      return;
+    }
+  }
   const int tx = threadIdx.x & 63, ty = threadIdx.x >> 6;
 #pragma unroll 4
   for (int r = ty; r < 64; r += 4) {
@@ -33,9 +66,10 @@
   if (n_tiles <= 0) return 0;
   hipStream_t st = (hipStream_t)stream;
   if (dtype == PF_F32)
-    k_seg_transpose<float><<<n_tiles, PF_THREADS, 0, st>>>((const float*)src_flat, (float*)dst_flat, (const PfTile*)tiles);
+    k_seg_transpose<float><<<n_tiles, PF_THREADS, 0, st>>>((const float*)src_flat, (float*)dst_flat, (const PfTile*)tiles, 0);
   else if (dtype == PF_BF16)
-    k_seg_transpose<bf16_t><<<n_tiles, PF_THREADS, 0, st>>>((const bf16_t*)src_flat, (bf16_t*)dst_flat, (const PfTile*)tiles);
+    k_seg_transpose<bf16_t><<<n_tiles, PF_THREADS, 0, st>>>((const bf16_t*)src_flat, (bf16_t*)dst_flat, (const PfTile*)tiles,
+                                                            pf_aligned16(src_flat) && pf_aligned16(dst_flat) ? 1 : 0);
   else
     return (int)hipErrorInvalidValue;
   PF_LAUNCH_CHECK();
diff --git a/pocketflow_amd/graph.py b/pocketflow_amd/graph.py
--- a/pocketflow_amd/graph.py
+++ b/pocketflow_amd/graph.py
@@ -262,10 +262,12 @@
     kh, kw, cin, cout = v.ref_shape
     return self.w_t[v.offset:v.offset + v.numel].view(cin, kh, kw, cout)
 
-  def zero_grad(self) -> None:
+  def zero_grad(self, w: bool = True, o: bool = True) -> None:
     if self.w_grad is not None:
-      self.w_grad.zero_()
-      self.o_grad.zero_()
+      if w:
+        self.w_grad.zero_()
+      if o:
+        self.o_grad.zero_()
 
   def weight_descs(self, variables: Sequence[Variable]) -> List[WeightDesc]:
     return [v.weight_desc() for v in variables]
diff --git a/pocketflow_amd/hip.py b/pocketflow_amd/hip.py
--- a/pocketflow_amd/hip.py
+++ b/pocketflow_amd/hip.py
@@ -50,6 +50,7 @@
     'pf_dw_i8_supported', 'pf_dw_i8_fwd',
     'pf_bn_act_quant_static', 'pf_conv_i8_fwd_q', 'pf_dw_i8_fwd_q',
     'pf_bn_add_act_groups', 'pf_bn_add_act_fwd', 'pf_bn_add_act_bwd_gate', 'pf_bn_add_act_bwd_gate_add',
+    'pf_adam_flat_zero', 'pf_momentum_flat_zero', 'pf_adam_flat_zero_dev', 'pf_momentum_flat_zero_dev',
 ]
 
 
@@ -242,6 +243,39 @@
   _check(_lib.pf_momentum_flat_dev(_ptr(p), _ptr(g), c_int(dtype_code(g)), _ptr(acc), _ptr(mask), c_int64(p.numel()),
                                    c_int64(int(n_decay)), c_float(wd), c_float(g_scale), _ptr(hp),
                                    c_float(momentum), _stream()), 'pf_momentum_flat_dev')
+
+
+
+def adam_flat_zero(p, g, m, v, mask, n_decay: int, wd: float, g_scale: float, lr: float, beta1: float,
+                   beta2: float, eps: float, beta1_power: float, beta2_power: float) -> None:
+  assert g.numel() == p.numel()
+  _check(_lib.pf_adam_flat_zero(_ptr(p), _ptr(g), c_int(dtype_code(g)), _ptr(m), _ptr(v), _ptr(mask),
+                                c_int64(p.numel()), c_int64(int(n_decay)), c_float(wd), c_float(g_scale), c_float(lr),
+                                c_float(beta1), c_float(beta2), c_float(eps), c_float(beta1_power),
+                                c_float(beta2_power), _stream()), 'pf_adam_flat_zero')
+
+
+def momentum_flat_zero(p, g, acc, mask, n_decay: int, wd: float, g_scale: float, lr: float,
+                       momentum: float) -> None:
+  assert g.numel() == p.numel()
+  _check(_lib.pf_momentum_flat_zero(_ptr(p), _ptr(g), c_int(dtype_code(g)), _ptr(acc), _ptr(mask), c_int64(p.numel()),
+                                    c_int64(int(n_decay)), c_float(wd), c_float(g_scale), c_float(lr),
+                                    c_float(momentum), _stream()), 'pf_momentum_flat_zero')
+
+
+def adam_flat_zero_dev(p, g, m, v, mask, n_decay: int, wd: float, g_scale: float, hp, beta1: float, beta2: float,
+                       eps: float) -> None:
+  assert g.numel() == p.numel()
+  _check(_lib.pf_adam_flat_zero_dev(_ptr(p), _ptr(g), c_int(dtype_code(g)), _ptr(m), _ptr(v), _ptr(mask),
+                                    c_int64(p.numel()), c_int64(int(n_decay)), c_float(wd), c_float(g_scale), _ptr(hp),
+                                    c_float(beta1), c_float(beta2), c_float(eps), _stream()), 'pf_adam_flat_zero_dev')
+
+
+def momentum_flat_zero_dev(p, g, acc, mask, n_decay: int, wd: float, g_scale: float, hp, momentum: float) -> None:
+  assert g.numel() == p.numel()
+  _check(_lib.pf_momentum_flat_zero_dev(_ptr(p), _ptr(g), c_int(dtype_code(g)), _ptr(acc), _ptr(mask), c_int64(p.numel()),
+                                        c_int64(int(n_decay)), c_float(wd), c_float(g_scale), _ptr(hp),
+                                        c_float(momentum), _stream()), 'pf_momentum_flat_zero_dev')
 
 
 def set_floats(dst, a: float, b: float = 0.0, c: float = 0.0, d: float = 0.0) -> None:
diff --git a/pocketflow_amd/optim.py b/pocketflow_amd/optim.py
--- a/pocketflow_amd/optim.py
+++ b/pocketflow_amd/optim.py
@@ -62,50 +62,59 @@
     self.g_scale = 1.0
     self.w_grad_src = self.o_grad_src = None
 
+  def _update_fn(self, name: str, own: bool):
+    fn = getattr(hip, name.replace('_flat', '_flat_zero'), None) if own else None
+    if fn is not None:
+      return fn, True
+    return getattr(hip, name), False
+
   def apply_gradients(self, lrn_rate: float) -> None:
     st = self.store
     wd = float(self.weight_decay)
     w_grad = self.w_grad_src if self.w_grad_src is not None else st.w_grad
     o_grad = self.o_grad_src if self.o_grad_src is not None else st.o_grad
+    dev = '_dev' if self.hp is not None else ''
+    fn_w, w_reset = self._update_fn(self.kind + '_flat' + dev, self.w_grad_src is None and st.w_size > 0)
+    fn_o, o_reset = self._update_fn(self.kind + '_flat' + dev, self.o_grad_src is None and st.o_size > 0)
     if self.hp is not None:
       if not self.hyper_external:
         self.feed_hyper(lrn_rate)
       if self.kind == 'adam':
         if st.w_size:
-          hip.adam_flat_dev(st.w_master, w_grad, self.slots_w[0], self.slots_w[1], self.w_mask, st.w_decay, wd, self.g_scale,
-                            self.hp, self.beta1, self.beta2, self.epsilon)
+          fn_w(st.w_master, w_grad, self.slots_w[0], self.slots_w[1], self.w_mask, st.w_decay, wd, self.g_scale,
+               self.hp, self.beta1, self.beta2, self.epsilon)
         if st.o_size:
-          hip.adam_flat_dev(st.o_master, o_grad, self.slots_o[0], self.slots_o[1], self.o_mask, st.o_decay, wd, self.g_scale,
-                            self.hp, self.beta1, self.beta2, self.epsilon)
+          fn_o(st.o_master, o_grad, self.slots_o[0], self.slots_o[1], self.o_mask, st.o_decay, wd, self.g_scale,
+               self.hp, self.beta1, self.beta2, self.epsilon)
       else:
         if st.w_size:
-          hip.momentum_flat_dev(st.w_master, w_grad, self.slots_w[0], self.w_mask, st.w_decay, wd, self.g_scale, self.hp,
-                                self.momentum)
+          fn_w(st.w_master, w_grad, self.slots_w[0], self.w_mask, st.w_decay, wd, self.g_scale, self.hp,
+               self.momentum)
         if st.o_size:
-          hip.momentum_flat_dev(st.o_master, o_grad, self.slots_o[0], self.o_mask, st.o_decay, wd, self.g_scale, self.hp,
-                                self.momentum)
+          fn_o(st.o_master, o_grad, self.slots_o[0], self.o_mask, st.o_decay, wd, self.g_scale, self.hp,
+               self.momentum)
       st.w_t_fresh = False
-      st.zero_grad()
+      st.zero_grad(w=not w_reset, o=not o_reset)
       return
     if self.kind == 'adam':
       b1p, b2p = float(self.beta1_power), float(self.beta2_power)
       if st.w_size:
-        hip.adam_flat(st.w_master, w_grad, self.slots_w[0], self.slots_w[1], self.w_mask, st.w_decay, wd,
-                      self.g_scale, lrn_rate, self.beta1, self.beta2, self.epsilon, b1p, b2p)
+        fn_w(st.w_master, w_grad, self.slots_w[0], self.slots_w[1], self.w_mask, st.w_decay, wd,
+             self.g_scale, lrn_rate, self.beta1, self.beta2, self.epsilon, b1p, b2p)
       if st.o_size:
-        hip.adam_flat(st.o_master, o_grad, self.slots_o[0], self.slots_o[1], self.o_mask, st.o_decay, wd,
-                      self.g_scale, lrn_rate, self.beta1, self.beta2, self.epsilon, b1p, b2p)
+        fn_o(st.o_master, o_grad, self.slots_o[0], self.slots_o[1], self.o_mask, st.o_decay, wd,
+             self.g_scale, lrn_rate, self.beta1, self.beta2, self.epsilon, b1p, b2p)
       self.beta1_power = np.float32(self.beta1_power * np.float32(self.beta1))
       self.beta2_power = np.float32(self.beta2_power * np.float32(self.beta2))
     else:
       if st.w_size:
-        hip.momentum_flat(st.w_master, w_grad, self.slots_w[0], self.w_mask, st.w_decay, wd, self.g_scale,
-                          lrn_rate, self.momentum)
+        fn_w(st.w_master, w_grad, self.slots_w[0], self.w_mask, st.w_decay, wd, self.g_scale,
+             lrn_rate, self.momentum)
       if st.o_size:
-        hip.momentum_flat(st.o_master, o_grad, self.slots_o[0], self.o_mask, st.o_decay, wd, self.g_scale,
-                          lrn_rate, self.momentum)
+        fn_o(st.o_master, o_grad, self.slots_o[0], self.o_mask, st.o_decay, wd, self.g_scale,
+             lrn_rate, self.momentum)
     st.w_t_fresh = False
-    st.zero_grad()
+    st.zero_grad(w=not w_reset, o=not o_reset)
 
 
 class GradReducer(object):
```
